# marbl/parsnp

Hardware: AMD Instinct MI355X
Metric: genomes/sec (MUM+LCB end-to-end) (higher is better)
Workload: dtype int32

## Files before the change

### parsnp_amd/csrc/engine/engine_core.h

```cpp
#pragma once
#include <algorithm>
#include <atomic>
#include <chrono>
#include <cstdint>
#include <cstdio>
#include <cstdlib>
#include <cstring>
#include <memory>
#include <mutex>
#include <new>
#include <string>
#include <thread>
#include <vector>

#include "kernels.h"
#include "store_kernels.h"
#include "dense_kernels.h"
#include "index_kernels.h"

namespace pm {

struct HostPool {
    void* (*alloc_fn)(size_t) = nullptr;
    void (*free_fn)(void*) = nullptr;
    struct Block { void* p = nullptr; size_t cap = 0; };
    std::vector<Block> idle;
    std::mutex mu;
    Block take(size_t n) {
        std::lock_guard<std::mutex> lk(mu);
        size_t best = idle.size();
        for (size_t i = 0; i < idle.size(); i++)
            if (idle[i].cap >= n && (best == idle.size() || idle[i].cap < idle[best].cap)) best = i;
        if (best != idle.size() && idle[best].cap <= 2 * n + (1u << 20)) { Block b = idle[best]; idle.erase(idle.begin() + (long)best); return b; }
        Block b; b.cap = n + n / 8 + 256; b.p = alloc_fn(b.cap);
        if (!b.p) throw std::bad_alloc();
        return b;
    }
    void give(Block b) { std::lock_guard<std::mutex> lk(mu); if (b.p) idle.push_back(b); }
    ~HostPool() { for (auto& b : idle) free_fn(b.p); }
};

struct ClearJob { void* p; size_t bytes; int value; };
struct BatchResult {
    int64_t nregions = 0, total = 0;
    int nq = 0;
    std::vector<int64_t> off;
    HostPool::Block kb, lonb, spb, fwdb;
    HostPool::Block startb, strandb, flagsb;
    bool rows = false, dirty_known = false;
    int64_t table_id = 0;
    int64_t store_base = -1;
    std::shared_ptr<HostPool> pool;
    int32_t* start() const { return (int32_t*)startb.p; }
    uint8_t* strand() const { return (uint8_t*)strandb.p; }
    const uint32_t* flags() const { return (const uint32_t*)flagsb.p; }
    const int32_t* k() const { return (const int32_t*)kb.p; }
    const int32_t* lon() const { return (const int32_t*)lonb.p; }
    const int32_t* sp() const { return (const int32_t*)spb.p; }
    const uint8_t* fwd() const { return (const uint8_t*)fwdb.p; }
    void release() {
        if (pool) { pool->give(kb); pool->give(lonb); pool->give(spb); pool->give(fwdb); pool->give(startb); pool->give(strandb); pool->give(flagsb); }
        kb = lonb = spb = fwdb = startb = strandb = flagsb = HostPool::Block();
    }
    BatchResult() = default;
    BatchResult(const BatchResult&) = delete;
    BatchResult& operator=(const BatchResult&) = delete;
    ~BatchResult() { release(); }
};

struct PhaseTime { const char* name; float ms; };

struct Collectives {
    int rank = 0, world = 1;
    int (*allreduce_min_i32)(void* ctx, int32_t* buf, int64_t count) = nullptr;
    int (*allgather)(void* ctx, const void* send, int64_t send_bytes, void* recv) = nullptr;
    void* ctx = nullptr;
    bool device = false;
};

inline int bits_for(uint64_t v) { int b = 1; while (b < 64 && (v >> b)) b++; return b; }

template <class B>
class Engine {
public:
    explicit Engine(B& backend) : be(backend), pool(std::make_shared<HostPool>()) { pool->alloc_fn = &B::host_alloc; pool->free_fn = &B::host_free; }
    std::shared_ptr<HostPool> pool;
    ~Engine() { release(); }

    std::string error;
    std::vector<PhaseTime> timing;
    int64_t last_events = 0, last_candidates = 0, last_rest = 0, last_positions = 0, last_accepted = 0;
    double last_alg[3] = {0, 0, 0};
    uint64_t alg_raw[3] = {0, 0, 0};
    uint64_t alg_sets[8 * kAlgSets] = {};

    int ngen = 0;
    bool want_rows = false;
    std::vector<int64_t> glen_h;
    Collectives coll;
    int g_first = 1, g_last = 1;
    void set_shard(const Collectives& c) { coll = c; }
    static void shard_range(int n, int rank, int world, int* first, int* last) {
        int q = n - 1;
        *first = 1 + (int)((int64_t)q * rank / world);
        *last = 1 + (int)((int64_t)q * (rank + 1) / world);
    }

    int load_genomes(int n, const uint8_t* const* seqs, const int64_t* lens) {
        const bool dbg = getenv("PARSNP_DEBUG_TIMERS") != nullptr;
        auto now = [] { return std::chrono::duration<double>(std::chrono::steady_clock::now().time_since_epoch()).count(); };
        double tl = now();
        auto lap = [&](const char* what) { if (dbg) { be.sync(); const double t = now(); fprintf(stderr, "[upload] %-14s %.4f s\n", what, t - tl); tl = t; } };
        ngen = n;
        glen_h.assign(lens, lens + n);
        shard_range(n, coll.rank, coll.world, &g_first, &g_last);
        auto resident = [&](int) { return true; };
        std::vector<int64_t> goff(2 * (size_t)n);
        int64_t words = 2;
        int64_t maxlen = 0;
        for (int g = 0; g < n; g++) {
            if (!resident(g)) { goff[2 * (size_t)g] = goff[2 * (size_t)g + 1] = 64; continue; }
            maxlen = std::max(maxlen, lens[g]);
            for (int s = 0; s < 2; s++) {
                goff[2 * (size_t)g + s] = words * 32;
                words += (lens[g] + 31) / 32 + 2;
            }
        }
        words += 8;
        total_words = words;
        blk = (SeqBlock*)be.alloc((size_t)words * sizeof(SeqBlock));
        d_goff = (int64_t*)be.alloc(sizeof(int64_t) * 2 * (size_t)n);
        d_glen = (int64_t*)be.alloc(sizeof(int64_t) * (size_t)n);
        if (!blk || !d_goff || !d_glen) { error = "device allocation failed (genomes)"; return -3; }
        lap("allocate");
        be.memset(blk, 0, (size_t)words * sizeof(SeqBlock));
        be.h2d(d_goff, goff.data(), sizeof(int64_t) * goff.size());
        be.h2d(d_glen, lens, sizeof(int64_t) * (size_t)n);
        std::vector<char> res((size_t)n, 0);
        for (int g = 0; g < n; g++) res[(size_t)g] = resident(g) && lens[g] > 0;
        lap("clear + tables");
        if (!be.stage_genomes(n, seqs, lens, res, goff, blk, maxlen)) { error = "genome upload failed: " + be.error(); return -3; }
        lap("stage + pack");
        P = Packed{blk, d_goff, d_glen};
        return 0;
    }

    std::vector<int64_t> mumi_covered;
    struct GapBatch {
        const int64_t* ref_start = nullptr; const int64_t* ref_len = nullptr;
        const int32_t* store_ids = nullptr;
    };
    int run(int64_t nreg, const int64_t* starts, const int64_t* lens, const int32_t* minsize, BatchResult* out, bool want_events = false,
            bool mumi = false, const GapBatch* gb = nullptr) {
        budget_exceeded = false;
        dense_mode = false; dense_h.clear(); last_dense_regions = 0; last_dense_overrun_ms = -1;
        const int64_t ordinal = call_ordinal;
        if (dense_all && nreg > 0) { dense_h.assign((size_t)nreg, 1); dense_mode = true; }
        const auto t0 = std::chrono::steady_clock::now();
        index_rebuild = false;
        int rc = run_once(nreg, starts, lens, minsize, out, want_events, mumi, gb);
        if (rc == kIndexRebuild) {
            (void)be.collect();
            call_ordinal = ordinal;
            index_rebuild = true;
            rc = run_once(nreg, starts, lens, minsize, out, want_events, mumi, gb);
        }
        if (rc == -5 && budget_exceeded && !dense_mode) {
            budget_retries++;
            last_dense_overrun_ms = (float)std::chrono::duration<double, std::milli>(std::chrono::steady_clock::now() - t0).count();
            dense_h.resize((size_t)nreg);
            be.d2h(dense_h.data(), d_dense.p, (size_t)nreg);
            (void)be.collect();
            call_ordinal = ordinal;
            dense_mode = true; budget_exceeded = false;
            rc = run_once(nreg, starts, lens, minsize, out, want_events, mumi, gb);
            if (rc == kIndexRebuild) {
                (void)be.collect();
                call_ordinal = ordinal;
                index_rebuild = true;
                rc = run_once(nreg, starts, lens, minsize, out, want_events, mumi, gb);
            }
        }
        dense_mode = false; index_rebuild = false;
        return rc;
    }
    bool dense_all = false;
    int64_t last_dense_regions = 0;
    float last_dense_overrun_ms = -1;
    int dense_rounds = 0;
    int64_t anchor_table_id = 0, anchor_table_rows = 0;
    bool budget_exceeded = false;
    long budget_retries = 0;
    static constexpr int kIndexRebuild = -99;
    bool index_rebuild = false;
    int64_t index_overflow_seen = 0;
    int run_once(int64_t nreg, const int64_t* starts, const int64_t* lens, const int32_t* minsize, BatchResult* out, bool want_events,
                 bool mumi, const GapBatch* gb = nullptr) {
        timing.clear();
        const int nq = ngen - 1;
        out->nregions = nreg; out->nq = nq; out->total = 0;
        out->off.assign((size_t)nreg + 1, 0);
        out->release();
        out->pool = pool;
        if (nreg == 0) return 0;
        if (nq < 1) { error = "need at least one query genome"; return -2; }
        const int no_small = mumi ? 1 : 0;

        const size_t nrow = (size_t)nreg * (size_t)ngen;
        const size_t regz = (size_t)nreg;
        const size_t bytes_R = sizeof(RegionInfo) * regz, bytes_pre = 8 * (regz + 1);
        const bool from_store = gb && gb->store_ids;
        if (gb && !from_store) { error = "bad region list"; return -2; }
        const size_t nrow_staged = gb ? 0 : nrow;
        uint8_t* block = (uint8_t*)be.staging(bytes_R + 2 * bytes_pre + 16 * nrow_staged + (gb ? 4 * regz : 0) + 64);
        if (!block) { error = "cannot allocate the request staging block"; return -3; }
        RegionInfo* R = (RegionInfo*)block;
        int64_t* posbase = (int64_t*)(block + bytes_R);
        int64_t* cbase = posbase + regz + 1;
        int64_t* stage = cbase + regz + 1;
        std::vector<size_t> guess_r(regz, 0);
        std::vector<int64_t> units_r(regz, 0);
        if (from_store) {
            for (int64_t r = 0; r < nreg; r++) {
                if (gb->store_ids[r] < 0 || gb->store_ids[r] >= rg_count) { error = "region outside the region store"; return -2; }
                if (gb->ref_start[r] < 0 || gb->ref_len[r] < 0 || gb->ref_start[r] + gb->ref_len[r] > glen_h[0]) { error = "region outside its genome"; return -2; }
                if (gb->ref_len[r] >= (1ll << 31)) { error = "region longer than 2^31"; return -5; }
            }
            memcpy(stage, gb->store_ids, sizeof(int32_t) * regz);
        } else {
            const int nt = (int)std::max<int64_t>(1, std::min<int64_t>(8, nreg / 512));
            std::vector<int> bad((size_t)nt, 0);
            auto part = [&](int t) {
                const int64_t r0 = nreg * t / nt, r1 = nreg * (t + 1) / nt;
                for (int64_t r = r0; r < r1; r++) {
                    const int64_t* st = starts + r * ngen; const int64_t* ln = lens + r * ngen;
                    const int minlen = minsize[r] < 1 ? 1 : minsize[r];
                    const int div = std::max(8, minlen);
                    const int K = minlen < kMaxK ? minlen : kMaxK, stride = minlen - K + 1;
                    const int64_t nR = ln[0];
                    size_t gs = 0;
                    int64_t units = 0;
                    int b = 0;
                    for (int g = 0; g < ngen; g++) {
                        if (st[g] < 0 || ln[g] < 0 || st[g] + ln[g] > glen_h[(size_t)g]) b |= 1;
                        if (ln[g] >= (1ll << 31)) b |= 2;
                        if (!g) continue;
                        gs += (size_t)(2 * ln[g] / div);
                        int64_t ns = (ln[g] >= K && nR >= K && g >= g_first && g < g_last) ? (ln[g] - K) / stride + 1 : 0;
                        if (small_pair(nR, ln[g]) && !no_small) ns = 0;
                        units += (ns + kUnitSamples - 1) / kUnitSamples;
                    }
                    guess_r[(size_t)r] = gs; units_r[(size_t)r] = units;
                    bad[(size_t)t] |= b;
                    memcpy(stage + r * ngen, st, sizeof(int64_t) * (size_t)ngen);
                    memcpy(stage + nrow + r * ngen, ln, sizeof(int64_t) * (size_t)ngen);
                }
            };
            if (nt == 1) part(0);
            else {
                std::vector<std::thread> th;
                for (int t = 1; t < nt; t++) th.emplace_back(part, t);
                part(0);
                for (auto& x : th) x.join();
            }
            int b = 0;
            for (int x : bad) b |= x;
            if (b & 1) { error = "region outside its genome"; return -2; }
            if (b & 2) { error = "region longer than 2^31"; return -5; }
        }
        int64_t npos = 0, tsize = 0, fwords = 0, nunits = 0;
        int64_t tsize_b = 0, fwords_b = 0, nbk = 0, npos_bucketed = 0;
        std::vector<int64_t> bbase(regz + 1, 0);
        const bool by_index_buckets = index_build && !index_rebuild;
        int32_t max_nr = 1;
        size_t ev_guess = 1 << 16;
        cbase[0] = 0;
        for (int64_t r = 0; r < nreg; r++) {
            RegionInfo& ri = R[(size_t)r];
            ri.ref_pos = gb ? gb->ref_start[r] : starts[r * ngen];
            ri.nR = (int32_t)(gb ? gb->ref_len[r] : lens[r * ngen]);
            ri.minsize = minsize[r];
            ri.minlen = minsize[r] < 1 ? 1 : minsize[r];
            ri.K = ri.minlen < kMaxK ? ri.minlen : kMaxK;
            ri.stride = ri.minlen - ri.K + 1;
            int64_t slots = 16;
            while (slots < slot_factor * (int64_t)ri.nR) slots <<= 1;
            ri.tmask = (uint32_t)(slots - 1);
            int64_t fbits = 64;
            while (fbits < filter_factor * (int64_t)ri.nR) fbits <<= 1;
            ri.fmask = (uint32_t)(fbits - 1);
            const int ls = bits_for((uint64_t)slots) - 1, lf = bits_for((uint64_t)fbits) - 1;
            const int sb = std::min(kBucketBits, ls - 1), fb = lf - (ls - sb);
            const bool bucketed = by_index_buckets && slots >= index_bucket_min && fb >= 5 && fb <= kBucketFilterBits;
            ri.pad_ = bucketed ? (uint32_t)sb | ((uint32_t)fb << 8) | kBucketed : (uint32_t)ls | ((uint32_t)std::min(lf, 29) << 8);
            bbase[(size_t)r] = nbk;
            if (bucketed) { nbk += slots >> sb; npos_bucketed += ri.nR; }
            ri.tbase = bucketed ? -1 - tsize_b : tsize; (bucketed ? tsize_b : tsize) += slots;
            ri.fbase = bucketed ? -1 - fwords_b : fwords; (bucketed ? fwords_b : fwords) += fbits / 32;
            ri.posbase = npos; posbase[(size_t)r] = npos; npos += ri.nR;
            cbase[(size_t)r + 1] = cbase[(size_t)r] + (((int64_t)ri.nR + kChunkPos - 1) >> kCoarseShift) + 1;
            max_nr = std::max(max_nr, ri.nR);
            ev_guess += guess_r[(size_t)r];
            nunits += units_r[(size_t)r];
        }
        posbase[regz] = npos;
        bbase[regz] = nbk;
        const int64_t tsize_clear = tsize, fwords_clear = fwords;
        for (int64_t r = 0; r < nreg; r++) {
            RegionInfo& ri = R[(size_t)r];
            if (ri.tbase < 0) { ri.tbase = tsize_clear + (-1 - ri.tbase); ri.fbase = fwords_clear + (-1 - ri.fbase); }
        }
        tsize += tsize_b; fwords += fwords_b;
        last_index_bucketed = npos_bucketed; last_index_overflow = index_rebuild ? index_overflow_seen : 0; last_index_lost = -1;
        last_positions = npos; last_candidates = 0; last_accepted = 0; last_grouped = 0; last_grouped_wide = 0; last_handed_back = -1; last_wide_regions = 0;
        const int64_t npairs = nreg * nq;
        const int64_t nchunks = cbase[regz] - nreg;
        const int64_t centries = cbase[regz] * nq;
        const int lbits = bits_for((uint64_t)max_nr);
        if (bits_for((uint64_t)npairs) + lbits + 1 > 64) { error = "batch too large for 64-bit event keys"; return -5; }
        if (npairs >= (1ll << 31) || nreg >= (1ll << 31)) { error = "too many regions in one batch"; return -5; }
        if (nunits >= (1ll << 31)) { error = "too many work units in one batch"; return -5; }
        if (centries >= (1ll << 31)) { error = "coarse event index too large"; return -5; }

        be.mark("setup");
        ensure(d_R, regz);
        ensure(d_starts, nrow); ensure(d_lens, nrow);
        ensure(d_posbase, regz + 1); ensure(d_cbase, regz + 1);
        be.h2d_staged(d_R.p, R, bytes_R);
        be.h2d_staged(d_posbase.p, posbase, bytes_pre);
        be.h2d_staged(d_cbase.p, cbase, bytes_pre);
        if (!gb) {
            be.h2d_staged(d_starts.p, stage, sizeof(int64_t) * nrow);
            be.h2d_staged(d_lens.p, stage + nrow, sizeof(int64_t) * nrow);
        } else if (from_store) {
            ensure(d_list, regz);
            be.h2d_staged(d_list.p, stage, sizeof(int32_t) * regz);
            be.launch("gather_regions", (int64_t)nrow, GatherRegions{d_list.p, ngen, d_rg_start.p, d_rg_len.p, d_starts.p, d_lens.p});
        }
        const size_t ncounter = (size_t)kSlices * kSliceStride + 8;
        ensure(d_counter, ncounter);
        uint32_t* d_err = (uint32_t*)(d_counter.p + (size_t)kSlices * kSliceStride);

        ensure(d_slots, (size_t)tsize); ensure(d_filter, (size_t)fwords);
        ensure(d_next, (size_t)std::max<int64_t>(npos, 1)); ensure(d_rep, (size_t)std::max<int64_t>(npos, 1));
        ensure(d_epm, (size_t)std::max<int64_t>(npos, 1) + 1);
        const int64_t nwv = (npos + 63) / 64;
        const bool from_store_ = gb && gb->store_ids;
        ensure(d_repeated, (size_t)(npos / 32 + 2));
        ensure(d_ucount, (size_t)npairs + 1); ensure(d_uoff, (size_t)npairs + 1);
        ensure(d_coarse, (size_t)std::max<int64_t>(centries, 1));
        ensure(d_wmask, (size_t)nwv + 1); ensure(d_wcount, (size_t)nwv + 1); ensure(d_woff, (size_t)nwv + 1);
        if (from_store_) ensure(d_alg, 8 * (size_t)kAlgSets);
        ensure(d_dense, regz);
        {
            const ClearJob jobs[] = {
                {d_filter.p, sizeof(uint32_t) * (size_t)fwords_clear, 0}, {d_slots.p, sizeof(uint64_t) * (size_t)tsize_clear, 0xff}, {d_counter.p, 8 * ncounter, 0},
                {d_repeated.p, 4 * (size_t)(npos / 32 + 2), 0}, {d_coarse.p, 4 * (size_t)std::max<int64_t>(centries, 1), 0},
                {d_ucount.p + npairs, 8, 0}, {d_wcount.p + nwv, 8, 0}, {from_store_ ? d_alg.p : nullptr, from_store_ ? (size_t)64 * kAlgSets : 0, 0},
                {dense_mode ? nullptr : d_dense.p, dense_mode ? 0 : regz, 0}};
            be.clear_many(jobs, (int)(sizeof jobs / sizeof jobs[0]));
        }
        int64_t nflag = 0;
        if (dense_mode) {
            for (int64_t r = 0; r < nreg; r++) nflag += dense_h[(size_t)r] ? 1 : 0;
            be.h2d(d_dense.p, dense_h.data(), regz);
            last_dense_regions = nflag;
        }
        if (gb) be.launch("check_rows", (int64_t)nrow, CheckRows{d_R.p, d_starts.p, d_lens.p, ngen, d_glen, d_err});
        last_alg[0] = last_alg[1] = last_alg[2] = 0;
        if (from_store) {
            be.launch_wave("alg_bytes", (nreg * nq + kAlgPairs - 1) / kAlgPairs, AlgBytes{d_R.p, d_lens.p, ngen, nreg * nq, d_alg.p});
        }
        be.mark("index");
        const size_t kOvfSlot = (size_t)kSlices * kSliceStride + 6, kLostSlot = kOvfSlot + 1;
        const uint64_t ovf_cap = nbk > 0 ? (uint64_t)(index_overflow_cap > 0 ? index_overflow_cap : npos_bucketed / 32 + 1024) : 0;
        if (nbk > 0) {
            const int pbits = bits_for((uint64_t)npos), bbits = bits_for((uint64_t)nbk);
            if (pbits + bbits > 64) { error = "batch too large for 64-bit index keys"; return -5; }
            ensure(d_bkbase, regz + 1); ensure(d_ikey, (size_t)npos); ensure(d_ikey2, (size_t)npos); ensure(d_bkbegin, (size_t)nbk + 1); ensure(d_ovf, (size_t)ovf_cap);
            be.h2d(d_bkbase.p, bbase.data(), 8 * (regz + 1));
            be.launch("index_keys", npos, IndexKeys{P, d_R.p, nreg, d_posbase.p, d_bkbase.p, pbits, d_ikey.p, d_next.p, d_rep.p});
            if (!sort_keys_on(be, d_ikey.p, d_ikey2.p, (size_t)npos, pbits, pbits + bbits, 0)) {
                ensure(d_ikey3, (size_t)npos); ensure(d_ikey4, (size_t)npos);
                be.launch("index_key_buckets", npos, IndexKeyBuckets{d_ikey.p, pbits, d_ikey3.p});
                be.sort_pairs(d_ikey3.p, d_ikey4.p, d_ikey.p, d_ikey2.p, (size_t)npos, bbits);
            }
            be.launch("index_bucket_bounds", nbk + 1, IndexBucketBounds{d_ikey2.p, npos, pbits, d_bkbegin.p});
            be.launch_wave("index_bucket_fill", nbk, IndexBucketFill{P, d_R.p, nreg, d_bkbase.p, d_ikey2.p, d_bkbegin.p, pbits, d_slots.p, d_filter.p, d_next.p, d_rep.p,
                                                                     d_counter.p + kOvfSlot, d_ovf.p, ovf_cap});
            be.launch("index_overflow", (int64_t)ovf_cap, IndexOverflow{P, d_R.p, nreg, d_posbase.p, d_counter.p + kOvfSlot, d_ovf.p, ovf_cap, d_slots.p, d_next.p, d_rep.p});
        }
        if (npos_bucketed < npos) be.launch("index_insert", npos, IndexInsert{P, d_R.p, nreg, d_posbase.p, d_slots.p, d_next.p, d_filter.p, d_rep.p});
        if (index_verify) be.launch("index_verify", npos, IndexVerify{P, d_R.p, nreg, d_posbase.p, d_slots.p, d_filter.p, d_next.p, d_counter.p + kLostSlot});
        bool index_counts_read = false;
        be.mark("repeat");
        ensure(d_run, (size_t)std::max<int64_t>(npos, 1));
        be.launch("run_length", npos, RunLength{P, d_R.p, nreg, d_posbase.p, d_run.p});
        be.launch("repeat_length", npos, RepeatLength{P, d_R.p, nreg, d_posbase.p, d_slots.p, d_filter.p, d_next.p, d_run.p, d_rep.p, d_repeated.p, d_err, work_budget, d_dense.p});
        if (nflag > 0) {
            be.mark("dense_sa");
            if (int rc = dense_build(R, nreg, nflag)) return rc;
        }

        be.mark("units");
        be.launch("count_units", npairs, CountUnits{d_R.p, d_lens.p, ngen, d_ucount.p, g_first, g_last, no_small});
        be.exclusive_scan(d_ucount.p, d_uoff.p, (size_t)npairs + 1);
        if (!gb && nreg == 1) call_ordinal = 0; else if (gb) call_ordinal++;
        const size_t ord = gb || nreg == 1 ? (size_t)call_ordinal : (size_t)-1;
        if (ord != (size_t)-1 && call_hints.size() <= ord) call_hints.resize(ord + 1);
        CallHint none;
        CallHint& hint = ord != (size_t)-1 ? call_hints[ord] : none;
        if (hint_shrink > 1) {
            if (hint.units > 0) hint.units = std::max<int64_t>(1, hint.units / hint_shrink);
            if (hint.ncand > 0) hint.ncand = std::max<int64_t>(1, hint.ncand / hint_shrink);
        }
        bool units_known = !gb;
        if (gb && !(fast_tail && hint.units > 0)) {
            be.d2h(&nunits, d_uoff.p + npairs, 8);
            units_known = true;
        } else if (gb) nunits = hint.units + hint.units / 8 + 64;
        if (nunits >= (1ll << 31)) { error = "too many work units in one batch"; return -5; }
        if (gb) ev_guess += (size_t)nunits * 16;

        ensure(d_sliceoff, (size_t)kSlices + 1);
        uint64_t nev = 0;
        size_t slice_cap = (std::min<size_t>(std::max<size_t>(ev_cap_hint, ev_guess), (size_t)1 << 31) + kSlices - 1) / kSlices + 64;
        std::vector<uint64_t> counts(ncounter);
        uint32_t errbits = 0;
        ensure(d_qcount, (size_t)kSlices * kSliceStride);
        size_t queue_cap = std::max<size_t>(std::max<size_t>(rest_cap_hint[nreg == 1], (size_t)nunits * kUnitSamples / 16 / kSlices), 64) + 64;
        uint64_t nrest = 0;
        uint32_t sticky = 0;
        std::vector<uint64_t> qcounts((size_t)kSlices * kSliceStride);
        const bool small_groups = group_small && !no_small && !want_events && nreg >= 2;
        const bool first_form = small_groups && nq <= kGrpGenomes;
        const bool wide_form = small_groups && group_wide && nq <= kWideGenomes;
        const bool grouping = first_form || wide_form;
        const size_t kGrpSlot = (size_t)kSlices * kSliceStride + 2;
        const size_t kWideSlot = kGrpSlot + 1;
        size_t grp_cap = grouping ? std::max<size_t>(grp_cap_hint, (size_t)npairs * 3) + 64 : 0;
        uint64_t ngrp = 0;
        if (grouping) { ensure(d_gflag, (size_t)nreg); ensure(d_glo, (size_t)npairs); }
        int64_t nunits_live = nunits;
        uint64_t worst_slice = 0;
        for (bool again = false;; again = true) {
            ensure(d_units, (size_t)std::max<int64_t>(nunits, 1));
            be.launch("fill_units", nunits, FillUnits{P, d_starts.p, d_lens.p, ngen, d_uoff.p, d_ucount.p, npairs, d_units.p});
            ensure(d_evkey, slice_cap * kSlices); ensure(d_evval, slice_cap * kSlices); ensure(d_rest, queue_cap * kSlices);
            if (again) be.memset(d_counter.p, 0, 8 * ncounter);
            if (grouping) {
                ensure(d_evkey3, grp_cap + ev_cap_hint); ensure(d_evval3, grp_cap + ev_cap_hint);
                ensure(d_state, grp_cap + ev_cap_hint); ensure(d_emax, grp_cap + ev_cap_hint);
                be.mark("grouped_events");
                if (first_form)
                    be.launch_wave("grouped_pair_events", xcd_grid(nreg),
                                   GroupedPairEvents{P, d_R.p, d_starts.p, d_lens.p, ngen, d_rep.p, d_evkey3.p, d_evval3.p, d_counter.p + kGrpSlot, (uint64_t)grp_cap, lbits,
                                                     d_glo.p, g_first, g_last, d_gflag.p, d_state.p, d_emax.p, d_epm.p, (int64_t)nreg});
                if (wide_form)
                    be.launch_wave("grouped_pair_events_wide", xcd_grid(nreg),
                                   GroupedPairEventsWide{P, d_R.p, d_starts.p, d_lens.p, ngen, d_rep.p, d_evkey3.p, d_evval3.p, d_counter.p + kGrpSlot, (uint64_t)grp_cap, lbits,
                                                         d_glo.p, g_first, g_last, d_gflag.p, d_state.p, d_emax.p, d_epm.p, (int64_t)nreg, first_form ? 1 : 0, d_counter.p + kWideSlot});
            }
            be.memset(d_qcount.p, 0, 8 * (size_t)kSlices * kSliceStride);
            be.mark("seed_extend");
            be.launch("seed_extend", nunits * 64,
                      SeedExtend{P, d_R.p, d_units.p, d_slots.p, d_filter.p, d_next.p, d_rep.p, d_repeated.p,
                                 d_evkey.p, d_evval.p, d_counter.p, (uint64_t)slice_cap, lbits, d_err, work_budget, d_rest.p, d_qcount.p, (uint64_t)queue_cap, d_uoff.p + npairs});
            if (nunits > 0)
                be.launch("seed_rest", (int64_t)(queue_cap * kSlices),
                          SeedRest{P, d_R.p, d_units.p, d_rest.p, d_qcount.p, (uint64_t)queue_cap, d_slots.p, d_filter.p, d_next.p, d_rep.p,
                                   d_evkey.p, d_evval.p, d_counter.p, (uint64_t)slice_cap, lbits, d_err, work_budget, d_dense.p});
            if (nunits > 0 && nflag > 0) {
                be.mark("dense_search");
                be.launch("seed_dense", (int64_t)(queue_cap * kSlices),
                          SeedDense{P, d_R.p, d_units.p, d_rest.p, d_qcount.p, (uint64_t)queue_cap, d_dfi.p, d_dstart.p, d_dval2.p, d_rep.p,
                                    d_evkey.p, d_evval.p, d_counter.p, (uint64_t)slice_cap, lbits});
                be.mark("seed_extend");
            }
            if (!no_small)
                be.launch("small_pair_events", npairs * 2,
                          SmallPairEvents{P, d_R.p, d_starts.p, d_lens.p, ngen, d_rep.p, d_evkey.p, d_evval.p, d_counter.p, (uint64_t)slice_cap, lbits, g_first, g_last, grouping ? d_gflag.p : nullptr});
            be.mark("sort");
            be.launch_wave("slice_offsets", 1, SliceOffsets{d_counter.p, d_sliceoff.p});
            group_downloads();
            be.d2h_async(qcounts.data(), d_qcount.p, 8 * qcounts.size());
            if (from_store) be.d2h_async(alg_sets, d_alg.p, sizeof alg_sets);
            if (!units_known) be.d2h_async(&nunits_live, d_uoff.p + npairs, 8);
            run_beside();
            be.d2h(counts.data(), d_counter.p, 8 * counts.size());
            if (!index_counts_read) {
                index_counts_read = true;
                if (nbk > 0) last_index_overflow = (int64_t)counts[kOvfSlot];
                if (index_verify) last_index_lost = (int64_t)counts[kLostSlot];
                if (nbk > 0 && counts[kOvfSlot] > ovf_cap) { index_overflow_seen = (int64_t)counts[kOvfSlot]; return kIndexRebuild; }
            }
            if (!units_known) {
                units_known = true;
                if (nunits_live >= (1ll << 31)) { error = "too many work units in one batch"; return -5; }
                if (nunits_live > nunits) {
                    nunits = nunits_live;
                    queue_cap = std::max<size_t>(queue_cap, (size_t)nunits * kUnitSamples / 16 / kSlices + 64);
                    tail_repeats++;
                    continue;
                }
            }
            uint64_t worst = 0, qworst = 0;
            nev = 0; nrest = 0;
            for (int sl = 0; sl < kSlices; sl++) {
                const uint64_t c = counts[(size_t)sl * kSliceStride]; nev += c; worst = std::max(worst, c);
                const uint64_t q = qcounts[(size_t)sl * kSliceStride]; nrest += q; qworst = std::max(qworst, q);
            }
            errbits = (uint32_t)counts[(size_t)kSlices * kSliceStride];
            ngrp = grouping ? counts[kGrpSlot] : 0;
            worst_slice = worst;
            if (worst <= slice_cap && qworst <= queue_cap && ngrp <= grp_cap) break;
            if (ngrp > grp_cap) grp_cap = (size_t)(ngrp + ngrp / 8 + 64);
            if (worst > slice_cap) slice_cap = (size_t)(worst + worst / 8 + 64);
            if (qworst > queue_cap) queue_cap = (size_t)(qworst + qworst / 8 + 64);
            sticky |= errbits & (kErrWork | kErrRows);
        }
        errbits |= sticky;
        if (from_store) {
            alg_raw[0] = alg_raw[1] = alg_raw[2] = 0;
            for (int x = 0; x < kAlgSets; x++) for (int k = 0; k < 3; k++) alg_raw[k] += alg_sets[8 * x + k];
        }
        if (from_store) { last_alg[0] = (double)alg_raw[0] / 4.0; last_alg[1] = (double)alg_raw[1] / 2.0; last_alg[2] = (double)alg_raw[2] / 2.0; }
        if (errbits & kErrRows) { error = "region outside its genome"; return -2; }
        rest_cap_hint[nreg == 1] = queue_cap - 64;
        if (gb) hint.units = std::max<int64_t>(nunits_live, 1);
        last_rest = (int64_t)nrest;
        ev_cap_hint = (size_t)(nev + nev / 4);
        if (grouping) grp_cap_hint = (size_t)(ngrp + ngrp / 4);
        last_events = (int64_t)(nev + ngrp);
        last_grouped = (int64_t)ngrp;
        last_grouped_wide = wide_form ? (int64_t)counts[kWideSlot] : 0;
        last_handed_back = wide_form ? (int64_t)counts[kWideSlot + 1] : -1;
        last_wide_regions = wide_form ? (int64_t)counts[kWideSlot + 2] : 0;
        const bool sharded = coll.world > 1 || coll.device;
        if ((errbits & kErrWork) && !sharded) { budget_exceeded = true; error = "per-thread work budget exceeded (degenerate repeat structure in a region)"; return -5; }

        ensure(d_evkey2, std::max<size_t>(nev, 1)); ensure(d_evval2, std::max<size_t>(nev, 1));
        ensure_keep(d_evkey3, std::max<size_t>(ngrp + nev, 1), (size_t)ngrp); ensure_keep(d_evval3, std::max<size_t>(ngrp + nev, 1), (size_t)ngrp);
        const int keybits = bits_for((uint64_t)npairs) + lbits + 1;
        uint64_t *skey = d_evkey3.p, *sval = d_evval3.p;
        const int64_t nbuckets = (int64_t)nq * nchunks;
        const bool by_buckets = bucket_sort && nev > 0 && nbuckets < ((int64_t)1 << 31);
        ensure(d_lo, (size_t)npairs + 1);
        if (by_buckets) {
            ensure(d_bcount, (size_t)nbuckets + 1); ensure(d_bbegin, (size_t)nbuckets + 1); ensure(d_pbase, (size_t)npairs);
            int shift = 6;
            while (((uint64_t)1 << shift) < worst_slice) shift++;
            be.memset(d_bcount.p, 0, 8 * ((size_t)nbuckets + 1));
            be.launch("pair_bucket_base", npairs, PairBucketBase{nq, d_cbase.p, d_pbase.p});
            be.launch("event_bucket_count", (int64_t)kSlices << shift, EventBucketCount{d_evkey.p, d_counter.p, (uint64_t)slice_cap, shift, lbits, d_pbase.p, d_bcount.p});
            be.exclusive_scan(d_bcount.p, d_bbegin.p, (size_t)nbuckets + 1);
            be.launch("event_place", (int64_t)kSlices << shift,
                      EventPlace{d_evkey.p, d_evval.p, d_counter.p, (uint64_t)slice_cap, shift, lbits, d_pbase.p, d_bbegin.p, d_bcount.p, d_evkey3.p + ngrp, d_evval3.p + ngrp});
            be.launch("event_order", nbuckets, EventOrder{d_bbegin.p, nbuckets, d_evkey3.p + ngrp, d_evval3.p + ngrp});
        } else if (nev > 0) {
            be.launch("compact_events", (int64_t)nev, CompactEvents{d_evkey.p, d_evval.p, d_sliceoff.p, (uint64_t)slice_cap, d_evkey2.p, d_evval2.p});
            be.sort_pairs(d_evkey2.p, d_evkey3.p + ngrp, d_evval2.p, d_evval3.p + ngrp, (size_t)nev, keybits);
        }
        be.mark("scan");
        const int64_t nev_sorted = (int64_t)nev;
        nev += ngrp;
        if (by_buckets) be.launch("coarse_from_buckets", centries, CoarseFromBuckets{d_bbegin.p, d_cbase.p, nreg, nq, (int64_t)ngrp, d_coarse.p, d_lo.p, npairs, nev_sorted});
        else be.launch("pair_bounds", npairs, PairBounds{skey, (int64_t)nev, lbits, npairs, d_lo.p, (int64_t)ngrp});
        if (grouping) be.launch("grouped_bounds", npairs, GroupedBounds{d_gflag.p, d_glo.p, nq, d_lo.p});
        ensure_keep(d_state, std::max<size_t>(nev, 1), (size_t)ngrp); ensure_keep(d_emax, std::max<size_t>(nev, 1), (size_t)ngrp);
        const int64_t nsorted = (int64_t)(nev - ngrp);
        if (nsorted > 0) {
            const int64_t nwaves = (nsorted + kWaveEvents - 1) / kWaveEvents;
            ensure(d_wsummary, (size_t)nwaves);
            const WaveScanCore core{skey + ngrp, sval + ngrp, nsorted, lbits, d_R.p, nq, d_rep.p};
            be.launch_wave("wave_summary", nwaves, WaveSummary{core, d_wsummary.p});
            be.launch_wave("wave_scan", nwaves, WaveScan{core, d_wsummary.p, d_lo.p, (int64_t)ngrp, d_state.p + ngrp, d_emax.p + ngrp});
        }

        if (want_events) {
            ev_key_h.resize((size_t)nev); ev_val_h.resize((size_t)nev); rep_h.resize((size_t)npos);
            if (nev) { be.d2h(ev_key_h.data(), skey, 8 * (size_t)nev); be.d2h(ev_val_h.data(), sval, 8 * (size_t)nev); }
            if (npos) be.d2h(rep_h.data(), d_rep.p, 4 * (size_t)npos);
            ev_lbits = lbits;
        }

        if (mumi) {
            be.mark("mumi_coverage");
            ensure(d_cov, (size_t)npairs);
            be.launch("mumi_coverage", npairs, MumiCoverage{d_R.p, skey, sval, d_lo.p, d_state.p, d_rep.p, lbits, ngen, d_cov.p});
            mumi_covered.resize((size_t)npairs);
            be.d2h(mumi_covered.data(), d_cov.p, 8 * (size_t)npairs);
            if (sharded) {
                int widest = 0;
                for (int r = 0; r < coll.world; r++) { int a, b; shard_range(ngen, r, coll.world, &a, &b); widest = std::max(widest, b - a); }
                const size_t per = (size_t)std::max(widest, 1) + 1;
                std::vector<int64_t> send(per, 0), recv(per * (size_t)coll.world);
                for (int g = g_first; g < g_last; g++) send[(size_t)(g - g_first)] = mumi_covered[(size_t)(g - 1)];
                send[per - 1] = errbits;
                if (allgather_host(send.data(), (int64_t)(8 * send.size()), recv.data())) { error = "all-gather of MUMi coverage failed"; return -4; }
                for (int r = 0; r < coll.world; r++) {
                    int a, b; shard_range(ngen, r, coll.world, &a, &b);
                    for (int g = a; g < b; g++) mumi_covered[(size_t)(g - 1)] = recv[(size_t)r * per + (size_t)(g - a)];
                    errbits |= (uint32_t)recv[(size_t)r * per + per - 1];
                }
                if (errbits & kErrWork) { budget_exceeded = true; error = "per-thread work budget exceeded on some rank (degenerate repeat structure in a region)"; return -5; }
            }
            be.mark(nullptr);
            collect_timing();
            return 0;
        }

        be.mark("master_ep");
        if (!by_buckets) be.launch("coarse_fill", (int64_t)nev, CoarseFill{skey, (int64_t)nev, lbits, d_lo.p, d_R.p, d_cbase.p, nq, d_coarse.p});
        else if (ngrp > 0) be.launch("coarse_fill", (int64_t)ngrp, CoarseFill{skey, (int64_t)ngrp, lbits, d_lo.p, d_R.p, d_cbase.p, nq, d_coarse.p});
        if (master_seg) be.launch_wave("master_ep_seg", xcd_grid(nchunks), MasterEPSeg{d_R.p, nreg, ngen, skey, d_lo.p, d_emax.p, lbits, d_epm.p, d_cbase.p, d_coarse.p, g_first, g_last, grouping ? d_gflag.p : nullptr, nchunks});
        else be.launch_wave("master_ep", xcd_grid(nchunks), MasterEP{d_R.p, nreg, ngen, skey, d_lo.p, d_emax.p, lbits, d_epm.p, d_cbase.p, d_coarse.p, g_first, g_last, grouping ? d_gflag.p : nullptr, nchunks});
        int32_t verdict = 0;
        if (sharded && coll.device) {
            be.mark("exchange_ep");
            be.fill32(d_epm.p + npos, (errbits & kErrWork) ? -1 : 0);
            if (be.allreduce_min_i32_dev(d_epm.p, npos + 1)) { error = "RCCL all-reduce of Master.EP failed: " + be.error(); return -4; }
            be.d2h_async(&verdict, d_epm.p + npos, 4);
        } else if (sharded) {
            be.mark("exchange_ep");
            std::vector<int32_t> h((size_t)npos + 1);
            if (npos) be.d2h(h.data(), d_epm.p, 4 * (size_t)npos);
            h[(size_t)npos] = (errbits & kErrWork) ? -1 : 0;
            if (coll.allreduce_min_i32(coll.ctx, h.data(), npos + 1)) { error = "all-reduce of Master.EP failed"; return -4; }
            verdict = h[(size_t)npos];
            if (verdict >= 0 && npos) be.h2d(d_epm.p, h.data(), 4 * (size_t)npos);
        }
        be.mark("candidates");
        be.launch_wave("cand_mark", nwv, CandMark{d_R.p, nreg, d_posbase.p, npos, d_epm.p, d_wmask.p, d_wcount.p});
        be.exclusive_scan(d_wcount.p, d_woff.p, (size_t)nwv + 1);
        const int64_t* ncand_p = d_woff.p + nwv;
        const bool anchor_guess = nreg == 1 && !gb && hint.nok >= dirty_min;
        const bool may_skip_waits = !sharded && want_rows && resident && hint.ncand > 0 && (from_store || anchor_guess) && fast_tail;
        for (int attempt = may_skip_waits ? 0 : 1;; attempt++) {
            const bool exact = attempt > 0;
            int64_t ncand_i = 0;
            if (exact) be.d2h(&ncand_i, ncand_p, 8);
            if (verdict < 0) { budget_exceeded = true; error = "per-thread work budget exceeded on some rank (degenerate repeat structure in a region)"; return -5; }
            if (exact) {
                last_candidates = ncand_i;
                if (ncand_i == 0) { hint.ncand = 1; hint.nok = 0; if (resident && from_store) out->store_base = ms_count; be.mark(nullptr); collect_timing(); return 0; }
            }
            const uint64_t ncand = exact ? (uint64_t)ncand_i : (uint64_t)(hint.ncand + hint.ncand / 8 + 256);
            ensure(d_cand, (size_t)ncand);
            be.launch("cand_write", nwv * 64, CandWrite{d_R.p, nreg, d_posbase.p, d_wmask.p, d_woff.p, d_cand.p, ncand});
            const uint64_t* scand = d_cand.p;

            be.mark("fold");
            ensure(d_ok, (size_t)ncand); ensure(d_ok_k, (size_t)ncand); ensure(d_ok_lon, (size_t)ncand);
            ensure(d_osp, (size_t)ncand * (size_t)nq); ensure(d_ofwd, (size_t)ncand * (size_t)nq);
            const GenomeAtK* at = nullptr;
            if (sharded) {
                ensure(d_at, (size_t)ncand * (size_t)nq);
                be.launch("state_at_candidate", (int64_t)ncand * nq, StateAtCandidate{d_R.p, scand, ngen, skey, sval, d_lo.p, d_state.p, d_rep.p, lbits, d_at.p, d_cbase.p, d_coarse.p});
                be.mark("exchange_states");
                const size_t nqz = (size_t)nq, cz = (size_t)ncand;
                int widest = 0;
                for (int r = 0; r < coll.world; r++) { int a, b; shard_range(ngen, r, coll.world, &a, &b); widest = std::max(widest, b - a); }
                widest = std::max(widest, 1);
                const size_t blk = cz * (size_t)widest;
                if (coll.device) {
                    ensure(d_xsend, blk); ensure(d_xrecv, blk * (size_t)coll.world);
                    be.launch("pack_states", (int64_t)blk, PackStates{d_at.p, nq, g_first - 1, g_last - g_first, widest, d_xsend.p});
                    if (be.allgather_dev(d_xsend.p, (int64_t)(sizeof(GenomeAtK) * blk), d_xrecv.p)) { error = "RCCL all-gather of candidate states failed: " + be.error(); return -4; }
                    be.launch("unpack_states", (int64_t)(cz * nqz), UnpackStates{d_xrecv.p, nq, coll.world, widest, (int64_t)ncand, d_at.p});
                } else {
                    std::vector<GenomeAtK> all(cz * nqz);
                    be.d2h(all.data(), d_at.p, sizeof(GenomeAtK) * all.size());
                    std::vector<GenomeAtK> send(blk), recv(blk * (size_t)coll.world);
                    const size_t mine = (size_t)(g_last - g_first);
                    for (size_t c = 0; c < cz; c++)
                        for (size_t x = 0; x < mine; x++) send[c * (size_t)widest + x] = all[c * nqz + (size_t)(g_first - 1) + x];
                    if (coll.allgather(coll.ctx, send.data(), (int64_t)(sizeof(GenomeAtK) * send.size()), recv.data())) { error = "all-gather of candidate states failed"; return -4; }
                    for (int r = 0; r < coll.world; r++) {
                        int a, b; shard_range(ngen, r, coll.world, &a, &b);
                        const GenomeAtK* src = recv.data() + (size_t)r * send.size();
                        for (size_t c = 0; c < cz; c++)
                            for (int x = 0; x < b - a; x++) all[c * nqz + (size_t)(a - 1 + x)] = src[c * (size_t)widest + (size_t)x];
                    }
                    be.h2d(d_at.p, all.data(), sizeof(GenomeAtK) * all.size());
                }
                be.mark("fold");
                at = d_at.p;
            }
            be.launch_wave("fold_candidates", xcd_grid((int64_t)ncand),
                           FoldCandidates{d_R.p, scand, ngen, at, skey, sval, d_lo.p, d_state.p, d_rep.p, lbits, d_cbase.p, d_coarse.p,
                                          d_ok_k.p, d_ok_lon.p, d_osp.p, d_ofwd.p, d_ok.p, (int64_t)ncand, ncand_p});

            be.mark("compact");
            ensure(d_okcnt, (size_t)ncand + 1); ensure(d_okpos, (size_t)ncand + 1);
            be.launch("ok_count", (int64_t)ncand + 1, OkCount{d_ok.p, ncand_p, d_okcnt.p, (int64_t)ncand});
            be.exclusive_scan(d_okcnt.p, d_okpos.p, (size_t)ncand + 1);
            const int64_t* nok_p = d_okpos.p + ncand;
            int64_t nok = 0;
            if (exact) be.d2h(&nok, nok_p, 8);
            const size_t nokz = exact ? (size_t)nok : (size_t)ncand, nqz2 = (size_t)nq, ngz = (size_t)ngen;
            ensure(d_creg, std::max<size_t>(nokz, 1)); ensure(d_ck, std::max<size_t>(nokz, 1)); ensure(d_clon, std::max<size_t>(nokz, 1));
            std::vector<int32_t> reg_h(nokz);
            out->release();
            out->kb = pool->take(4 * nokz); out->lonb = pool->take(4 * nokz);
            out->rows = want_rows; out->dirty_known = false; out->table_id = 0; out->store_base = -1;
            const int64_t ms_before = ms_count, rg_before = rg_count, lay_before = layout_rows, pkey_before = rg_pkey_init;
            bool anchor_call = false;
            if (!want_rows) {
                ensure(d_csp, std::max<size_t>(nokz * nqz2, 1)); ensure(d_cfwd, std::max<size_t>(nokz * nqz2, 1));
                be.launch("compact_sp", (int64_t)ncand * nq,
                          CompactSp{scand, d_ok.p, d_okpos.p, nq, d_ok_k.p, d_ok_lon.p, d_osp.p, d_ofwd.p, d_creg.p, d_ck.p, d_clon.p, d_csp.p, d_cfwd.p, ncand_p});
                be.mark("download");
                group_downloads();
                out->spb = pool->take(4 * nokz * nqz2); out->fwdb = pool->take(nokz * nqz2);
                be.d2h_async(out->spb.p, d_csp.p, 4 * nokz * nqz2);
                be.d2h_async(out->fwdb.p, d_cfwd.p, nokz * nqz2);
            } else {
                anchor_call = nreg == 1 && !gb && (exact ? nok >= dirty_min : anchor_guess);
                const bool keep_rows = resident && (anchor_call || from_store);
                const bool to_store = anchor_call || keep_rows;
                int32_t* p_start; uint8_t* p_strand; int32_t* p_lon; uint32_t* p_flags;
                if (to_store) {
                    if (anchor_call) { ms_count = 0; rg_count = 0; layout_rows = -1; rg_pkey_init = 0; }
                    const size_t base = (size_t)ms_count, upto = base + nokz;
                    ensure_keep(d_anchor_start, std::max<size_t>(upto * ngz, 1), base * ngz); ensure_keep(d_ms_strand, std::max<size_t>(upto * ngz, 1), base * ngz);
                    ensure_keep(d_anchor_lon, std::max<size_t>(upto, 1), base); ensure_keep(d_anchor_flags, std::max<size_t>(upto, 1), base);
                    ensure_keep(d_ms_shift, std::max<size_t>(upto, 1), base); ensure_keep(d_ms_len, std::max<size_t>(upto, 1), base); ensure_keep(d_ms_state, std::max<size_t>(upto, 1), base);
                    p_start = d_anchor_start.p + base * ngz; p_strand = d_ms_strand.p + base * ngz; p_lon = d_anchor_lon.p + base; p_flags = d_anchor_flags.p + base;
                    out->store_base = (int64_t)base;
                    ms_count = (int64_t)upto;
                } else {
                    ensure(d_csp, std::max<size_t>(nokz * ngz, 1)); ensure(d_cfwd, std::max<size_t>(nokz * ngz, 1)); ensure(d_cflags, std::max<size_t>(nokz, 1));
                    p_start = d_csp.p; p_strand = d_cfwd.p; p_lon = d_clon.p; p_flags = d_cflags.p;
                }
                const bool long_list = nreg == 1 && (exact ? nok >= dirty_min : anchor_guess);
                if (long_list) ensure(d_dirty, nokz);
                {
                    const ClearJob jobs[] = {{p_flags, 4 * nokz, 0}, {long_list ? d_dirty.p : nullptr, long_list ? 4 * nokz : 0, 0},
                                             {to_store ? d_ms_shift.p + (ms_count - (int64_t)nokz) : nullptr, to_store ? 4 * nokz : 0, 0},
                                             {to_store ? d_ms_state.p + (ms_count - (int64_t)nokz) : nullptr, to_store ? nokz : 0, 0}};
                    be.clear_many(jobs, 4);
                }
                be.launch("compact_candidates", (int64_t)ncand * ngen,
                          CompactCandidates{scand, d_ok.p, d_okpos.p, ngen, d_ok_k.p, d_ok_lon.p, d_osp.p, d_ofwd.p, d_starts.p, d_lens.p, d_glen,
                                            d_creg.p, d_ck.p, p_lon, p_start, p_strand, p_flags, ncand_p});
                if (long_list) {
                    const int64_t nblocks = ((int64_t)nokz + kDirtyBlock - 1) / kDirtyBlock, groups = (ngen + 63) / 64;
                    ensure(d_bmax, (size_t)nblocks * ngz); ensure(d_bmin, (size_t)nblocks * ngz);
                    be.launch_wave("dirty_extent", nblocks * groups, DirtyExtent{p_start, p_lon, p_flags, nok_p, ngen, d_bmax.p, d_bmin.p});
                    be.launch_wave("dirty_prefix", groups, DirtyPrefix{nblocks, ngen, d_bmax.p, d_bmin.p});
                    be.launch_wave("dirty_mark", nblocks * groups, DirtyMark{p_start, p_lon, nok_p, ngen, d_bmax.p, d_bmin.p, p_flags, d_dirty.p});
                    be.launch("dirty_merge", (int64_t)nokz, DirtyMerge{d_dirty.p, p_flags, nok_p});
                    out->dirty_known = true;
                }
                if (to_store) {
                    be.d2d(d_ms_len.p + (ms_count - (int64_t)nokz), p_lon, 4 * nokz);
                    if (anchor_call) out->table_id = ++table_counter;
                }
                be.mark("download");
                group_downloads();
                out->flagsb = pool->take(4 * nokz);
                be.d2h_async(out->flagsb.p, p_flags, 4 * nokz);
                if (!keep_rows) {
                    out->startb = pool->take(4 * nokz * ngz); out->strandb = pool->take(nokz * ngz);
                    be.d2h_async(out->startb.p, p_start, 4 * nokz * ngz);
                    be.d2h_async(out->strandb.p, p_strand, nokz * ngz);
                }
                be.d2h_async(out->lonb.p, p_lon, 4 * nokz);
            }
            if (!want_rows) be.d2h_async(out->lonb.p, d_clon.p, 4 * nokz);
            be.d2h_async(reg_h.data(), d_creg.p, 4 * nokz);
            be.d2h_async(out->kb.p, d_ck.p, 4 * nokz);
            int64_t counts_h[2] = {ncand_i, nok};
            if (!exact) { be.d2h_async(&counts_h[0], ncand_p, 8); be.d2h_async(&counts_h[1], nok_p, 8); }
            flush_downloads();
            be.mark(nullptr);
            be.sync();
            if (!exact) {
                ncand_i = counts_h[0]; nok = counts_h[1];
                const bool fits = (uint64_t)ncand_i <= ncand && anchor_call == (nreg == 1 && !gb && nok >= dirty_min);
                if (!fits) {
                    ms_count = ms_before; rg_count = rg_before; layout_rows = lay_before; rg_pkey_init = pkey_before;
                    tail_repeats++;
                    be.mark("candidates");
                    continue;
                }
                last_candidates = ncand_i;
                if (out->store_base >= 0) ms_count = out->store_base + nok;
            }
            hint.ncand = std::max<int64_t>(ncand_i, 1); hint.nok = nok;
            last_accepted = nok;
            if (anchor_call) { anchor_table_rows = nok; anchor_table_id = out->table_id; }
            for (int64_t w = 0; w < nok; w++) out->off[(size_t)reg_h[(size_t)w] + 1]++;
            for (int64_t r = 0; r < nreg; r++) out->off[(size_t)r + 1] += out->off[(size_t)r];
            out->total = out->off[(size_t)nreg];
            if (out->table_id && out->store_base == 0) anchor_flags_h.assign(out->flags(), out->flags() + nok);
            break;
        }
        collect_timing();
        return 0;
    }


    bool resident = false;
    int64_t ms_count = 0;
    int64_t rg_count = 0;
    std::vector<RegInfo> rg_info_h;
    std::vector<uint32_t> anchor_flags_h;
    static constexpr int kAgain = -6;

    void begin_store_call() { timing.clear(); last_events = last_rest = last_positions = last_candidates = last_accepted = last_grouped = last_grouped_wide = last_wide_regions = 0; last_handed_back = -1; last_index_bucketed = last_index_overflow = 0; last_index_lost = -1; last_alg[0] = last_alg[1] = last_alg[2] = 0; }
    Store store_view() { return Store{d_anchor_start.p, d_ms_strand.p, d_anchor_lon.p, d_anchor_flags.p, d_ms_shift.p, d_ms_len.p, d_ms_state.p, ngen}; }
    Layout layout_view(uint64_t* image, bool coherent = true) { return Layout{image, d_lay_off.p, d_lay_bits.p, coherent ? 1 : 0}; }
    size_t layout_geometry() {
        const size_t ngz = (size_t)ngen;
        if (lay_words == 0) {
            std::vector<int64_t> off(ngz + 1, 0), bits(ngz);
            for (size_t j = 0; j < ngz; j++) { bits[j] = glen_h[j] + 1; off[j + 1] = off[j] + (bits[j] + 63) / 64 + 1; }
            ensure(d_lay_off, ngz + 1); ensure(d_lay_bits, ngz);
            be.h2d(d_lay_off.p, off.data(), 8 * (ngz + 1)); be.h2d(d_lay_bits.p, bits.data(), 8 * ngz);
            lay_words = (size_t)off[ngz];
            lay_off_h = off;
        }
        return lay_words;
    }
    int need_resident(int64_t table_id) {
        if (!resident) { error = "the session is not in resident mode"; return -2; }
        if (table_id == 0 || table_id != anchor_table_id) { error = "the anchor table of this request is no longer resident"; return -2; }
        return 0;
    }
    int store_settle(int64_t table_id, RowInfo* out) {
        if (int rc = settle_launch(table_id)) return rc;
        return store_info(0, anchor_table_rows, out);
    }
    int settle_launch(int64_t table_id) {
        if (int rc = need_resident(table_id)) return rc;
        begin_store_call();
        const int64_t rows = anchor_table_rows;
        const size_t words = layout_geometry();
        ensure(d_image, words);
        be.mark("settle");
        ensure(d_foreign_count, 2);
        be.memset(d_foreign_count.p, 0, 16);
        ms_key_rows = 0; foreign_seen = 0;
        be.memset(d_image.p, 0, 8 * words);
        ensure(d_recwords, words);
        be.memset(d_recwords.p, 0, words);
        const Store S = store_view();
        const Layout L = layout_view(d_image.p);
        be.launch_wave("settle_clean", rows, SettleClean{S, P});
        std::vector<int32_t> fl;
        for (int64_t c = 0; c < rows; c++) { const uint32_t f = anchor_flags_h[(size_t)c]; if (!(f & (kRowBad | kRowOutside)) && (f & kRowDirty)) fl.push_back((int32_t)c); }
        const bool many_flagged = flagged_div > 1 && fl.size() * (size_t)flagged_div > (size_t)rows;
        bool ordered = true;
        for (int64_t c = 0; c < rows && ordered; c++) { const uint32_t f = anchor_flags_h[(size_t)c]; ordered = !((f & kRowEarly) && !(f & (kRowBad | kRowOutside | kRowDirty))); }
        if (ordered && !force_atomic_marks) be.launch_wave("store_mark_ordered", ((rows + kMarkRows - 1) / kMarkRows) * ((ngen + 63) / 64), StoreMarkOrdered{S, L, rows});
        else be.launch("store_mark", rows * ngen, StoreMark{S, L, 0, (uint8_t)(kStAccepted | kStFlagged), kStAccepted});
        be.launch("layout_sentinel", (int64_t)ngen, LayoutSentinel{d_lay_off.p, d_lay_bits.p, d_image.p});
        if (!fl.empty()) {
            const uint64_t* before_once = d_once.p; const uint64_t* before_twice = d_twice.p;
            ensure(d_once, words); ensure(d_twice, words); ensure(d_list, fl.size());
            if (d_once.p != before_once || d_twice.p != before_twice) { be.memset(d_once.p, 0, 8 * words); be.memset(d_twice.p, 0, 8 * words); }
            be.h2d(d_list.p, fl.data(), 4 * fl.size());
            be.launch("collide_mark", (int64_t)fl.size() * ngen, CollideMark{S, d_list.p, layout_view(d_once.p), d_twice.p});
            be.launch_wave("collide_test", (int64_t)fl.size(), CollideTest{S, d_list.p, layout_view(d_twice.p, false)});
            be.launch("collide_clear", (int64_t)fl.size() * ngen, CollideClear{S, d_list.p, layout_view(d_once.p), d_twice.p});
            ensure(d_t_rem, 2); ensure(d_t_done, fl.size());
            {
                const ClearJob jobs[] = {{d_t_rem.p, 16, 0}, {d_t_done.p, fl.size(), 0}};
                be.clear_many(jobs, 2);
            }
            be.launch("count_tangled", (int64_t)fl.size(), CountTangled{S, d_list.p, d_t_rem.p});
            if (many_flagged) {
                uint64_t tangled = 0;
                be.d2h(&tangled, d_t_rem.p, 8);
                if ((int64_t)tangled > tangled_max) {
                    be.mark(nullptr);
                    collect_timing_more();
                    error = "too many rows of the list overlap one another (rearranged genomes): the host route decides";
                    return kAgain;
                }
            }
            be.launch_wave("settle_flagged", (int64_t)fl.size(), SettleFlagged{S, layout_view(d_image.p, false), P, d_list.p});
            {
                const int32_t* before = d_owner.p;
                ensure(d_owner, words);
                if (d_owner.p != before) be.memset(d_owner.p, 0, 4 * words);
            }
            int rounds = tangle_rounds ? kTangleRounds : 0;
            if (rounds && tangle_ran > 0) {
                int last = 0;
                for (int r = 1; r < tangle_ran; r++) if (tangle_left[r] < tangle_left[r - 1]) last = r;
                rounds = std::min(kTangleRounds, last + 2);
            }
            ensure(d_t_left, kTangleRounds);
            for (int round = 0; round < rounds; round++) {
                be.launch_wave("tangle_owner", (int64_t)fl.size(), TangleOwner{S, d_list.p, d_lay_off.p, d_lay_bits.p, d_owner.p, d_t_done.p, d_t_rem.p});
                be.launch_wave("tangle_settle", (int64_t)fl.size(), TangleSettle{S, layout_view(d_image.p, false), P, d_list.p, d_owner.p, d_t_done.p, d_t_rem.p});
                be.launch_wave("tangle_clear", (int64_t)fl.size(), TangleClear{S, d_list.p, d_lay_off.p, d_lay_bits.p, d_owner.p, d_t_done.p, d_t_rem.p, d_t_left.p + round});
            }
            tangle_ran = 0;
            if (rounds) { be.d2h_async(tangle_left, d_t_left.p, 8 * (size_t)rounds); tangle_ran = rounds; }
            be.launch_wave("settle_tangled", 1, SettleTangled{S, L, P, d_list.p, (int64_t)fl.size(), d_t_done.p, d_t_rem.p});
        }
        layout_rows = rows;
        return 0;
    }
    int store_settle_seeds(int64_t table_id, int32_t q, RowInfo* out, std::vector<RegInfo>* infos, std::vector<int32_t>* ids) {
        infos->clear(); ids->clear();
        if (int rc = settle_launch(table_id)) return rc;
        const int64_t rows = anchor_table_rows;
        rg_count = 0;
        if (rows == 0) return 0;
        const Store S = store_view();
        ensure(d_rowinfo, (size_t)rows);
        be.launch("store_info", rows, StoreInfoOut{S, 0, d_rowinfo.p});
        be.mark("seeds");
        ensure(d_ch_flag, (size_t)rows + 1); ensure(d_ch_pos, (size_t)rows + 1); ensure(d_list, (size_t)rows);
        ensure(d_sd_cnt, (size_t)rows + 1); ensure(d_sd_off, (size_t)rows + 1); ensure(d_sd_keep, (size_t)rows);
        be.launch("chain_flag", rows + 1, ChainFlag{S, rows, d_ch_flag.p});
        be.exclusive_scan(d_ch_flag.p, d_ch_pos.p, (size_t)rows + 1);
        be.launch("anchor_list", rows, AnchorList{S, d_ch_pos.p, d_list.p});
        const int64_t* nacc = d_ch_pos.p + rows;
        const Layout L = layout_view(d_image.p, false);
        be.memset(d_sd_cnt.p + rows, 0, 8);
        be.launch_wave("seed_count", xcd_grid(rows), SeedCount{S, L, P, d_list.p, nacc, q, d_sd_cnt.p, d_sd_keep.p, rows});
        be.exclusive_scan(d_sd_cnt.p, d_sd_off.p, (size_t)rows + 1);
        size_t cap = std::max<size_t>(rg_cap_hint, (size_t)rows / 4 + 1024);
        std::vector<RegInfo> raw;
        for (bool again = false;; again = true) {
            ensure(d_rg_start, cap * (size_t)ngen); ensure(d_rg_len, cap * (size_t)ngen); ensure(d_rg_info, cap);
            be.launch_wave("seed_place", xcd_grid(rows), SeedPlace{S, L, P, d_list.p, nacc, d_sd_off.p, d_sd_keep.p, d_rg_start.p, d_rg_len.p, d_rg_info.p, (uint64_t)cap, rows});
            be.mark(nullptr);
            const size_t guess = std::min(cap, rg_cap_hint / (size_t)hint_shrink);
            raw.resize(guess);
            group_downloads();
            if (guess) be.d2h_async(raw.data(), d_rg_info.p, sizeof(RegInfo) * guess);
            if (!again) be.d2h_async(out, d_rowinfo.p, sizeof(RowInfo) * (size_t)rows);
            int64_t got = 0;
            be.d2h(&got, d_sd_off.p + rows, 8);
            if ((size_t)got <= cap) {
                rg_count = got;
                raw.resize((size_t)got);
                if ((size_t)got > guess) be.d2h(raw.data() + guess, d_rg_info.p + guess, sizeof(RegInfo) * ((size_t)got - guess));
                break;
            }
            cap = (size_t)got + (size_t)got / 8 + 64;
            be.mark("seeds");
        }
        rg_cap_hint = (size_t)rg_count + (size_t)rg_count / 4;
        if (rg_info_h.size() < (size_t)rg_count) rg_info_h.resize((size_t)rg_count);
        bool sorted = true;
        for (int64_t i = 0; i < rg_count; i++) { rg_info_h[(size_t)i] = raw[(size_t)i]; if (i && raw[(size_t)i - 1].key >= raw[(size_t)i].key) sorted = false; }
        if (!sorted) { error = "seed regions out of order"; return -4; }
        infos->swap(raw);
        ids->resize((size_t)rg_count);
        for (int64_t i = 0; i < rg_count; i++) (*ids)[(size_t)i] = (int32_t)i;
        collect_timing_more();
        return 0;
    }
    int store_info(int64_t first, int64_t count, RowInfo* out) {
        if (!resident || first < 0 || count < 0 || first + count > ms_count) { error = "rows outside the MUM store"; return -2; }
        if (count == 0) return 0;
        ensure(d_rowinfo, (size_t)count);
        be.launch("store_info", count, StoreInfoOut{store_view(), first, d_rowinfo.p});
        be.mark(nullptr);
        be.d2h(out, d_rowinfo.p, sizeof(RowInfo) * (size_t)count);
        collect_timing_more();
        return 0;
    }
    void take_regions(int64_t first, int64_t upto, std::vector<RegInfo>* infos, std::vector<int32_t>* ids) {
        const size_t m = (size_t)(upto - first);
        std::vector<RegInfo> raw(m);
        if (m) be.d2h(raw.data(), d_rg_info.p + first, sizeof(RegInfo) * m);
        if (rg_info_h.size() < (size_t)upto) rg_info_h.resize((size_t)upto);
        std::vector<int32_t> order;
        for (size_t i = 0; i < m; i++) { rg_info_h[(size_t)first + i] = raw[i]; if (raw[i].key >= 0) order.push_back((int32_t)i); }
        std::sort(order.begin(), order.end(), [&](int32_t x, int32_t y) { return raw[(size_t)x].key < raw[(size_t)y].key; });
        infos->clear(); ids->clear();
        for (int32_t i : order) { infos->push_back(raw[(size_t)i]); ids->push_back((int32_t)(first + i)); }
    }
    int store_seeds(int64_t table_id, const int32_t* acc, int64_t nacc, int32_t q, std::vector<RegInfo>* infos, std::vector<int32_t>* ids) {
        if (int rc = need_resident(table_id)) return rc;
        if (layout_rows < 0) { error = "the anchor list has not been settled"; return -2; }
        for (int64_t i = 0; i < nacc; i++) if (acc[i] < 0 || acc[i] >= anchor_table_rows) { error = "anchor outside the table"; return -2; }
        rg_count = 0;
        infos->clear(); ids->clear();
        begin_store_call();
        if (nacc == 0) return 0;
        ensure(d_list, (size_t)nacc); ensure(d_rg_count, 2);
        be.h2d(d_list.p, acc, 4 * (size_t)nacc);
        be.mark("seeds");
        size_t cap = std::max<size_t>(rg_cap_hint, (size_t)nacc / 4 + 1024);
        for (;;) {
            ensure(d_rg_start, cap * (size_t)ngen); ensure(d_rg_len, cap * (size_t)ngen); ensure(d_rg_info, cap);
            be.memset(d_rg_count.p, 0, 16);
            be.launch_wave("seed_walk", xcd_grid(nacc), SeedWalk{store_view(), layout_view(d_image.p, false), P, d_list.p, q, d_rg_start.p, d_rg_len.p, d_rg_info.p, d_rg_count.p, (uint64_t)cap, (int64_t)nacc});
            uint64_t got = 0;
            be.d2h(&got, d_rg_count.p, 8);
            if (got <= cap) { rg_count = (int64_t)got; break; }
            cap = (size_t)got + (size_t)got / 8 + 64;
        }
        rg_cap_hint = (size_t)rg_count + (size_t)rg_count / 4;
        be.mark(nullptr);
        take_regions(0, rg_count, infos, ids);
        collect_timing_more();
        return 0;
    }
    int store_regions_equal(const int32_t* a, const int32_t* b, int64_t n, uint8_t* same) {
        if (!resident) { error = "the session is not in resident mode"; return -2; }
        for (int64_t i = 0; i < n; i++) if (a[i] < 0 || a[i] >= rg_count || b[i] < 0 || b[i] >= rg_count) { error = "region outside the region store"; return -2; }
        if (n == 0) return 0;
        ensure(d_list, (size_t)n); ensure(d_list2, (size_t)n); ensure(d_small8, (size_t)n);
        be.h2d(d_list.p, a, 4 * (size_t)n); be.h2d(d_list2.p, b, 4 * (size_t)n);
        be.launch_wave("regions_equal", n, RegionsEqual{d_list.p, d_list2.p, ngen, d_rg_start.p, d_rg_len.p, d_small8.p});
        be.d2h(same, d_small8.p, (size_t)n);
        return 0;
    }
    void (*beside_fn)(void*) = nullptr; void* beside_ctx = nullptr;
    void run_beside() { if (beside_fn) { void (*f)(void*) = beside_fn; beside_fn = nullptr; f(beside_ctx); } }
    int store_search(const int32_t* ids, const int32_t* minsize, int64_t n, int64_t* first_row, int64_t* off, void (*beside)(void*) = nullptr, void* ctx = nullptr) {
        beside_fn = beside; beside_ctx = ctx;
        struct Always { Engine* e; ~Always() { e->run_beside(); } } on_every_way_out{this};
        if (!resident) { error = "the session is not in resident mode"; return -2; }
        std::vector<int64_t> rs((size_t)n), rl((size_t)n);
        for (int64_t i = 0; i < n; i++) {
            if (ids[i] < 0 || ids[i] >= rg_count) { error = "region outside the region store"; return -2; }
            rs[(size_t)i] = rg_info_h[(size_t)ids[i]].ref_start; rl[(size_t)i] = rg_info_h[(size_t)ids[i]].ref_len;
        }
        *first_row = ms_count;
        off[0] = 0;
        if (n == 0) return 0;
        GapBatch gb;
        gb.store_ids = ids; gb.ref_start = rs.data(); gb.ref_len = rl.data();
        BatchResult br;
        const bool keep = want_rows;
        want_rows = true;
        const int rc = run(n, nullptr, nullptr, minsize, &br, false, false, &gb);
        want_rows = keep;
        if (rc) return rc;
        *first_row = br.store_base >= 0 ? br.store_base : ms_count;
        for (int64_t i = 0; i <= n; i++) off[i] = br.off[(size_t)i];
        return 0;
    }
    int store_validate(const int32_t* regions, const int64_t* row0, const int32_t* cnt, int64_t nreg, const int64_t* cluster_first, int64_t ncl, int32_t q,
                       uint32_t* trouble, std::vector<RegInfo>* kids, std::vector<int32_t>* kid_ids, int64_t info_first = 0, int64_t info_count = 0, RowInfo* info = nullptr,
                       int64_t stage_first = 0, int32_t* second_stage_ran = nullptr, int32_t generation_no = 1, int32_t* done = nullptr) {
        if (!resident || layout_rows < 0) { error = "the anchor list has not been settled"; return -2; }
        kids->clear(); kid_ids->clear(); *trouble = 0;
        if (nreg == 0 || ncl == 0) return 0;
        int64_t total = 0;
        for (int64_t x = 0; x < nreg; x++) {
            if (regions[x] < 0 || regions[x] >= rg_count || row0[x] < 0 || cnt[x] < 0 || row0[x] + cnt[x] > ms_count) { error = "bad generation list"; return -2; }
            total += cnt[x];
        }
        if (cluster_first[0] != 0 || cluster_first[ncl] != nreg) { error = "bad cluster list"; return -2; }
        if (stage_first < 0 || stage_first >= ncl) { error = "bad stage boundary"; return -2; }
        begin_store_call();
        const size_t cap = (size_t)rg_count + 2 * (size_t)total + 16;
        ensure_keep(d_rg_start, cap * (size_t)ngen, (size_t)rg_count * (size_t)ngen); ensure_keep(d_rg_len, cap * (size_t)ngen, (size_t)rg_count * (size_t)ngen);
        ensure_keep(d_rg_info, cap, (size_t)rg_count);
        const size_t bytes = 4 * (size_t)nreg + 8 * (size_t)nreg + 4 * (size_t)nreg + 8 * ((size_t)ncl + 1) + 64;
        uint8_t* block = (uint8_t*)be.staging(bytes);
        if (!block) { error = "cannot allocate the request staging block"; return -3; }
        int64_t* s_row0 = (int64_t*)block; int64_t* s_first = s_row0 + nreg; int32_t* s_reg = (int32_t*)(s_first + ncl + 1); int32_t* s_cnt = s_reg + nreg;
        memcpy(s_row0, row0, 8 * (size_t)nreg); memcpy(s_first, cluster_first, 8 * ((size_t)ncl + 1)); memcpy(s_reg, regions, 4 * (size_t)nreg); memcpy(s_cnt, cnt, 4 * (size_t)nreg);
        ensure(d_v_row0, (size_t)nreg); ensure(d_v_first, (size_t)ncl + 1); ensure(d_list, (size_t)nreg); ensure(d_list2, (size_t)nreg); ensure(d_rg_count, 4);
        ensure(d_v_done, (size_t)ncl); ensure(d_v_defer, (size_t)ncl); ensure(d_v_involved, (size_t)ncl);
        be.h2d_staged(d_v_row0.p, s_row0, 8 * (size_t)nreg); be.h2d_staged(d_v_first.p, s_first, 8 * ((size_t)ncl + 1));
        be.h2d_staged(d_list.p, s_reg, 4 * (size_t)nreg); be.h2d_staged(d_list2.p, s_cnt, 4 * (size_t)nreg);
        foreign_cap = std::min<size_t>((size_t)1 << 16, ((size_t)32 << 20) / (8 * (size_t)ngen));
        ensure(d_foreign, foreign_cap); ensure(d_foreign_masks, foreign_cap * (size_t)ngen); ensure(d_foreign_count, 2);
        ensure_keep(d_ms_key, (size_t)ms_count, (size_t)ms_key_rows); ms_key_rows = ms_count;
        if (rg_pkey_init > rg_count) rg_pkey_init = 0;
        ensure_keep(d_rg_pkey, cap, (size_t)rg_pkey_init);
        if (rg_pkey_init < rg_count) { be.memset(d_rg_pkey.p + rg_pkey_init, 0, 8 * (size_t)(rg_count - rg_pkey_init)); rg_pkey_init = rg_count; }
        constexpr size_t kOutwCap = 4096; constexpr int64_t kOutwWaves = 256;
        ensure(d_outw, kOutwCap); ensure(d_outw_count, 2);
        const int64_t na = stage_first > 0 ? stage_first : ncl;
        uint64_t head[4] = {(uint64_t)rg_count, 0, 0, 0};
        if (info_count > 0) {
            if (info_first < 0 || info_first + info_count > ms_count) { error = "rows outside the MUM store"; return -2; }
            ensure(d_rowinfo, (size_t)info_count);
        }
        std::vector<int32_t> done_h((size_t)ncl, 0);
        auto generation = [&](bool exact) {
            be.h2d(d_rg_count.p, head, 32);
            be.memset(d_v_done.p, 0, 4 * (size_t)ncl);
            be.memset(d_outw_count.p, 0, 16);
            const uint8_t* defer = nullptr;
            if (exact) {
                be.memset(d_v_defer.p, 0, (size_t)ncl);
                const int64_t c0 = stage_first > 0 ? na : 0, cn = ncl - c0;
                if (cn >= 2) {
                    const size_t words = layout_geometry();
                    const uint64_t* b1 = d_once.p; const uint64_t* b2 = d_twice.p; const int32_t* b3 = d_owner.p;
                    ensure(d_once, words); ensure(d_twice, words); ensure(d_owner, words);
                    if (d_once.p != b1 || d_twice.p != b2) { be.memset(d_once.p, 0, 8 * words); be.memset(d_twice.p, 0, 8 * words); }
                    if (d_owner.p != b3) be.memset(d_owner.p, 0, 4 * words);
                    be.launch_wave("cluster_extents", cn, ClusterExtents{ngen, d_rg_start.p, d_rg_len.p, d_list.p, d_v_first.p, layout_view(d_once.p), d_twice.p, d_owner.p, c0, 1});
                    be.launch_wave("cluster_involved", cn, ClusterInvolved{ngen, d_rg_start.p, d_rg_len.p, d_list.p, d_v_first.p, layout_view(d_twice.p, false), d_owner.p, d_v_involved.p, c0});
                    be.launch_wave("cluster_defer", cn, ClusterDefer{ngen, d_rg_start.p, d_rg_len.p, d_list.p, d_v_first.p, d_lay_off.p, d_lay_bits.p, d_owner.p, d_v_involved.p, d_v_defer.p, c0});
                    be.launch_wave("cluster_extents", cn, ClusterExtents{ngen, d_rg_start.p, d_rg_len.p, d_list.p, d_v_first.p, layout_view(d_once.p), d_twice.p, d_owner.p, c0, 0});
                    int32_t* owner2 = (int32_t*)d_twice.p;
                    be.launch_wave("reader_mark", cn, ReaderMark{store_view(), d_v_row0.p, d_list2.p, ngen, d_rg_start.p, d_rg_len.p, d_list.p, d_v_first.p, layout_view(d_once.p), d_owner.p, owner2, c0, 1});
                    be.launch_wave("marker_look", cn, MarkerLook{store_view(), d_v_row0.p, d_list2.p, ngen, d_v_first.p, layout_view(d_once.p, false), d_owner.p, owner2, d_v_defer.p, c0});
                    be.launch_wave("reader_look", cn, ReaderLook{store_view(), d_v_row0.p, d_list2.p, ngen, d_rg_start.p, d_rg_len.p, d_list.p, d_v_first.p, d_lay_off.p, d_lay_bits.p, owner2, d_v_defer.p, c0});
                    be.launch_wave("reader_mark", cn, ReaderMark{store_view(), d_v_row0.p, d_list2.p, ngen, d_rg_start.p, d_rg_len.p, d_list.p, d_v_first.p, layout_view(d_once.p), d_owner.p, owner2, c0, 0});
                }
                defer = d_v_defer.p;
                exact_cluster_tests++;
            } else be.launch_wave("clusters_disjoint", ncl - 1, ClustersDisjoint{ngen, d_rg_start.p, d_rg_len.p, d_list.p, d_v_first.p, d_rg_count.p + 3, stage_first, force_unsure ? 1 : 0});
            be.launch_wave("cluster_validate", xcd_grid(na),
                           ClusterValidate{store_view(), layout_view(d_image.p), P, d_rg_start.p, d_rg_len.p, d_rg_info.p, d_rg_count.p, (uint64_t)cap,
                                           d_list.p, d_v_row0.p, d_list2.p, d_v_first.p, q, (uint32_t*)(d_rg_count.p + 1), na, 0, nullptr, d_rg_count.p + 3,
                                           d_foreign.p, d_foreign_count.p, (uint64_t)foreign_cap, d_foreign_masks.p, d_ms_key.p, generation_no, d_recwords.p, defer, d_v_done.p,
                                           d_rg_pkey.p, d_outw.p, d_outw_count.p, (uint64_t)kOutwCap});
            if (stage_first > 0) {
                be.launch("stage_gate", 1, StageGate{d_rg_count.p, (uint64_t)rg_count, force_gate ? 1 : 0});
                be.launch_wave("cluster_validate", xcd_grid(ncl - na),
                               ClusterValidate{store_view(), layout_view(d_image.p), P, d_rg_start.p, d_rg_len.p, d_rg_info.p, d_rg_count.p, (uint64_t)cap,
                                               d_list.p, d_v_row0.p, d_list2.p, d_v_first.p, q, (uint32_t*)(d_rg_count.p + 1), ncl - na, na, d_rg_count.p + 2, d_rg_count.p + 3,
                                               d_foreign.p, d_foreign_count.p, (uint64_t)foreign_cap, d_foreign_masks.p, d_ms_key.p, generation_no + 1, d_recwords.p, defer, d_v_done.p,
                                               d_rg_pkey.p, d_outw.p, d_outw_count.p, (uint64_t)kOutwCap});
            }
            be.launch_wave("outside_write_check", kOutwWaves,
                           OutsideWriteCheck{store_view(), d_rg_start.p, d_rg_len.p, d_rg_info.p, d_rg_pkey.p, d_rg_count.p, (uint64_t)cap, d_list.p, d_outw.p, d_outw_count.p, (uint64_t)kOutwCap,
                                             d_ms_key.p, anchor_table_rows, (uint32_t*)(d_rg_count.p + 1), kOutwWaves});
            if (info_count > 0) be.launch("store_info", info_count, StoreInfoOut{store_view(), info_first, d_rowinfo.p});
            be.mark(nullptr);
            group_downloads();
            if (info_count > 0) be.d2h_async(info, d_rowinfo.p, sizeof(RowInfo) * (size_t)info_count);
            be.d2h_async(&foreign_seen, d_foreign_count.p, 8);
            be.d2h_async(&outside_writes_call, d_outw_count.p, 8);
            be.d2h_async(done_h.data(), d_v_done.p, 4 * (size_t)ncl);
            be.d2h(head, d_rg_count.p, 32);
        };
        be.mark("validate");
        generation(clusters_out_of_order);
        if (head[3] != 0 && !clusters_out_of_order) {
            clusters_out_of_order = true;
            head[0] = (uint64_t)rg_count; head[1] = head[2] = head[3] = 0;
            be.mark("validate");
            generation(true);
        }
        *trouble = (uint32_t)head[1];
        outside_writes += (int64_t)outside_writes_call;
        const bool ran2 = stage_first > 0 && head[2] == 0;
        if (second_stage_ran) *second_stage_ran = ran2 ? 1 : 0;
        for (int64_t cl = 0; cl < ncl; cl++) {
            if (stage_first > 0 && cl >= na && !ran2) { done_h[(size_t)cl] = 0; continue; }
            const int64_t size = cluster_first[cl + 1] - cluster_first[cl];
            if (done_h[(size_t)cl] < size) {
                deferred_regions += size - done_h[(size_t)cl];
                if (!done && !*trouble) *trouble |= done_h[(size_t)cl] == 0 ? 8u : 1u;
            }
        }
        if (done) memcpy(done, done_h.data(), 4 * (size_t)ncl);
        if (head[0] > cap) { error = "region store overflow"; return -4; }
        const int64_t before = rg_count;
        rg_count = (int64_t)head[0];
        take_regions(before, rg_count, kids, kid_ids);
        collect_timing_more();
        return 0;
    }
    int store_judge(const int32_t* cur, const int32_t* back, int64_t n, int32_t d, int32_t* min_gap, int32_t* max_gap, uint8_t* verdict) {
        if (!resident) { error = "the session is not in resident mode"; return -2; }
        for (int64_t i = 0; i < n; i++) if (cur[i] < 0 || cur[i] >= ms_count || back[i] < 0 || back[i] >= ms_count) { error = "rows outside the MUM store"; return -2; }
        if (n == 0) return 0;
        begin_store_call();
        ensure(d_list, (size_t)n); ensure(d_list2, (size_t)n); ensure(d_j_min, (size_t)n); ensure(d_j_max, (size_t)n); ensure(d_small8, (size_t)n);
        int32_t* block = (int32_t*)be.staging(8 * (size_t)n);
        if (!block) { error = "cannot allocate the request staging block"; return -3; }
        memcpy(block, cur, 4 * (size_t)n); memcpy(block + n, back, 4 * (size_t)n);
        be.h2d_staged(d_list.p, block, 4 * (size_t)n); be.h2d_staged(d_list2.p, block + n, 4 * (size_t)n);
        be.mark("judge");
        be.launch_wave("judge_pairs", n, JudgePairs{store_view(), d_list.p, d_list2.p, d, d_j_min.p, d_j_max.p, d_small8.p});
        be.mark(nullptr);
        be.d2h_async(min_gap, d_j_min.p, 4 * (size_t)n); be.d2h_async(max_gap, d_j_max.p, 4 * (size_t)n);
        be.d2h(verdict, d_small8.p, (size_t)n);
        collect_timing_more();
        return 0;
    }
    int store_unmark(const int32_t* rows, int64_t n) {
        if (!resident || layout_rows < 0) { error = "the anchor list has not been settled"; return -2; }
        for (int64_t i = 0; i < n; i++) if (rows[i] < 0 || rows[i] >= ms_count) { error = "rows outside the MUM store"; return -2; }
        if (n == 0) return 0;
        ensure(d_list, (size_t)n);
        be.h2d(d_list.p, rows, 4 * (size_t)n);
        be.launch("store_unmark", n * ngen, StoreUnmark{store_view(), layout_view(d_image.p), d_list.p});
        return 0;
    }
    int store_fill(const int32_t* last_of, const int32_t* first_of_next, int64_t n, uint8_t* add, std::vector<int64_t>* starts, std::vector<int64_t>* ends) {
        if (!resident || layout_rows < 0) { error = "the anchor list has not been settled"; return -2; }
        for (int64_t i = 0; i < n; i++) if (last_of[i] < 0 || last_of[i] >= ms_count || first_of_next[i] < 0 || first_of_next[i] >= ms_count) { error = "rows outside the MUM store"; return -2; }
        starts->clear(); ends->clear();
        if (n == 0) return 0;
        begin_store_call();
        const size_t ngz = (size_t)ngen;
        ensure(d_list, (size_t)n); ensure(d_list2, (size_t)n); ensure(d_small8, (size_t)n); ensure(d_f_start, (size_t)n * ngz); ensure(d_f_end, (size_t)n * ngz);
        be.h2d(d_list.p, last_of, 4 * (size_t)n); be.h2d(d_list2.p, first_of_next, 4 * (size_t)n);
        be.mark("fill");
        be.launch_wave("fill_between", n, FillBetween{store_view(), layout_view(d_image.p, false), P, d_list.p, d_list2.p, d_small8.p, d_f_start.p, d_f_end.p});
        be.mark(nullptr);
        be.d2h(add, d_small8.p, (size_t)n);
        std::vector<int32_t> which;
        for (int64_t i = 0; i < n; i++) if (add[i] == 1) which.push_back((int32_t)i);
        if (!which.empty()) {
            const size_t m = which.size();
            ensure(d_list, m); ensure(d_f_pack, 2 * m * ngz);
            be.h2d(d_list.p, which.data(), 4 * m);
            be.launch("fill_gather", (int64_t)m * ngen, FillGather{d_list.p, ngen, d_f_start.p, d_f_end.p, d_f_pack.p});
            std::vector<int64_t> pack(2 * m * ngz);
            be.d2h(pack.data(), d_f_pack.p, 8 * pack.size());
            starts->resize(m * ngz); ends->resize(m * ngz);
            for (size_t k = 0; k < m; k++) {
                memcpy(starts->data() + k * ngz, pack.data() + (2 * k) * ngz, 8 * ngz);
                memcpy(ends->data() + k * ngz, pack.data() + (2 * k + 1) * ngz, 8 * ngz);
            }
        }
        collect_timing_more();
        return 0;
    }
    struct ChainInfo { int64_t n_in, lcbs_first, lcbs_dissolved, mums_dissolved, n_mums, n_lcbs, n_fillers; uint64_t trouble; };
    void order_check_launch(uint32_t* word, uint32_t bit) {
        const int64_t cnt = (int64_t)std::min<uint64_t>(foreign_seen, (uint64_t)foreign_cap);
        const int64_t rows = ms_count - layout_rows;
        if (cnt <= 0 || rows <= 0) return;
        ensure(d_hits, kHitCap); ensure(d_hit_count, 2); ensure(d_hit_owned, kHitCap * (size_t)ngen); ensure(d_hit_present, kHitCap * (size_t)ngen);
        be.memset(d_hit_count.p, 0, 16);
        const Store S = store_view();
        const Layout L = layout_view(d_image.p, false);
        be.launch_wave("foreign_bound", cnt, ForeignBound{S, L, P, d_rg_start.p, d_rg_len.p, d_foreign.p, cnt, d_foreign_masks.p, d_recwords.p, d_hits.p, d_hit_count.p, (uint64_t)kHitCap,
                                                         d_hit_owned.p, d_hit_present.p, word, bit});
        const int64_t chunks = (rows + kScanRows - 1) / kScanRows, waves = 8192;
        be.launch_wave("foreign_scan", waves, ForeignScan{S, d_rg_start.p, d_rg_len.p, d_ms_key.p, d_foreign.p, d_hits.p, d_hit_count.p, (uint64_t)kHitCap, d_hit_owned.p, d_hit_present.p,
                                                         layout_rows, ms_count, chunks, waves});
        be.launch_wave("foreign_decide_hits", (int64_t)kHitCap, ForeignDecideHits{S, L, P, d_rg_start.p, d_rg_len.p, d_foreign.p, d_foreign_masks.p, d_hits.p, d_hit_count.p, (uint64_t)kHitCap,
                                                                                 d_hit_owned.p, d_hit_present.p, word, bit});
        if (order_debug) {
            uint64_t nh = 0;
            be.d2h(&nh, d_hit_count.p, 8);
            fprintf(stderr, "[order check] %ld noted candidates, %ld left to the scan (launched for %ld), %ld recursion rows\n", (long)cnt, (long)nh, (long)kHitCap, (long)rows);
        }
    }
    int store_order_check(uint32_t* trouble) {
        if (!resident || layout_rows < 0) { error = "the anchor list has not been settled"; return -2; }
        *trouble = 0;
        begin_store_call();
        ensure(d_rg_count, 4);
        be.mark("validate");
        be.memset(d_rg_count.p + 1, 0, 8);
        order_check_launch((uint32_t*)(d_rg_count.p + 1), 1u);
        be.mark(nullptr);
        uint64_t word = 0;
        be.d2h(&word, d_rg_count.p + 1, 8);
        *trouble = (uint32_t)word;
        collect_timing_more();
        return 0;
    }
    int store_chain_begin(int64_t expect, int32_t d, float diag_diff, int64_t c) {
        if (!resident || layout_rows < 0) { error = "the anchor list has not been settled"; return -2; }
        if (expect <= 0 || expect > ms_count) { error = "bad MUM count"; return -2; }
        if (chain_event) { be.event_wait(chain_event); be.event_release(chain_event); chain_event = nullptr; }
        begin_store_call();
        const size_t rows = (size_t)ms_count, cap = (size_t)expect;
        ensure(d_ch_flag, rows + 1); ensure(d_ch_pos, rows + 1);
        ensure(d_ch_key, cap); ensure(d_ch_val, cap); ensure(d_ch_skey, cap); ensure(d_ch_srow, cap); ensure(d_ch_key2, cap); ensure(d_ch_row2, cap);
        ensure(d_ch_verdict, cap); ensure(d_ch_head, cap + 1); ensure(d_ch_hpos, cap + 1); ensure(d_ch_survive, cap + 1); ensure(d_ch_spos, cap + 1);
        ensure(d_ch_lcblen, cap); ensure(d_ch_hdr, kChWords); ensure(d_ch_outrow, cap); ensure(d_ch_outhead, cap);
        const size_t host_bytes = 8 * (size_t)kChWords + 4 * cap + cap;
        if (host_bytes > chain_host_cap) {
            if (chain_host) be.pinned_free(chain_host);
            chain_host_cap = 0;
            chain_host = (uint8_t*)be.pinned_alloc(host_bytes + host_bytes / 4 + 64);
            if (!chain_host) { error = "cannot allocate the chain result block"; return -3; }
            chain_host_cap = host_bytes + host_bytes / 4 + 64;
        }
        chain_cap = (int64_t)cap;
        const Store S = store_view();
        be.mark("chain");
        {
            const ClearJob jobs[] = {{d_ch_hdr.p, 8 * (size_t)kChWords, 0}, {d_ch_lcblen.p, 8 * cap, 0}};
            be.clear_many(jobs, 2);
        }
        order_check_launch((uint32_t*)(d_ch_hdr.p + kChTrouble), (uint32_t)kChainOrder);
        be.launch("chain_flag", (int64_t)rows + 1, ChainFlag{S, (int64_t)rows, d_ch_flag.p});
        be.exclusive_scan(d_ch_flag.p, d_ch_pos.p, rows + 1);
        be.launch("chain_keys", (int64_t)rows, ChainKeys{S, d_ch_pos.p, d_ch_key.p, d_ch_val.p, (int64_t)cap});
        be.sort_pairs(d_ch_key.p, d_ch_skey.p, d_ch_val.p, d_ch_srow.p, cap, bits_for((uint64_t)glen_h[0]));
        const int64_t* n1 = d_ch_pos.p + rows;
        int64_t* hdr = d_ch_hdr.p;
        uint64_t* trouble = (uint64_t*)(hdr + kChTrouble);
        const bool bp = diag_diff > 1.0f;
        int64_t* back = nullptr;
        if (bp) {
            ensure(d_ch_back, cap); ensure(d_ch_wflag, cap + 1); ensure(d_ch_wpos, cap + 1); ensure(d_ch_wend, cap); ensure(d_ch_wverdict, cap);
            ensure(d_ch_wlist, (size_t)kChainStarts); ensure(d_ch_wkeep, (size_t)kChainStarts);
            back = d_ch_back.p;
        }
        const int64_t nstarts = std::min<int64_t>((int64_t)cap, kChainStarts);
        auto windows = [&](const uint64_t* row, const int64_t* n) {
            be.launch("chain_starts", (int64_t)cap + 1, ChainHeads{d_ch_verdict.p, n, d_ch_wflag.p, kChPass});
            be.exclusive_scan(d_ch_wflag.p, d_ch_wpos.p, cap + 1);
            be.launch_wave("chain_window", (int64_t)cap, ChainWindow{S, row, n, d, diag_diff, d_ch_verdict.p, chain_window, d_ch_wpos.p, d_ch_wlist.p, d_ch_wend.p, d_ch_wverdict.p});
            be.launch("chain_select", 1, ChainSelect{n, d_ch_wpos.p, d_ch_wlist.p, d_ch_wend.p, d_ch_wkeep.p, trouble});
            be.launch_wave("chain_window_fill", nstarts, ChainWindowFill{n, d_ch_wpos.p, d_ch_wlist.p, d_ch_wend.p, d_ch_wverdict.p, d_ch_wkeep.p, trouble, d_ch_verdict.p, back});
        };
        be.launch_wave("chain_judge", (int64_t)cap, ChainJudge{S, d_ch_skey.p, d_ch_srow.p, n1, d, diag_diff, d_ch_verdict.p, trouble, force_chain_tie ? 1 : 0, back});
        be.launch("chain_judge_reverse", (int64_t)cap, ChainJudgeReverse{S, d_ch_srow.p, n1, d, diag_diff, d_ch_verdict.p});
        if (bp) windows(d_ch_srow.p, n1);
        be.launch("chain_heads", (int64_t)cap + 1, ChainHeads{d_ch_verdict.p, n1, d_ch_head.p, kChClose});
        be.exclusive_scan(d_ch_head.p, d_ch_hpos.p, cap + 1);
        be.launch("chain_lcb_sum", (int64_t)cap, ChainLcbSum{S, d_ch_srow.p, n1, d_ch_hpos.p, d_ch_verdict.p, d_ch_lcblen.p, hdr});
        be.launch("chain_dissolve", (int64_t)cap + 1, ChainDissolve{n1, d_ch_hpos.p, d_ch_head.p, d_ch_verdict.p, d_ch_lcblen.p, c, d_ch_survive.p, hdr});
        if (!bp) be.launch_wave("chain_unmark", (int64_t)cap, ChainUnmark{S, layout_view(d_image.p), d_ch_srow.p, n1, d_ch_survive.p, nullptr});
        be.exclusive_scan(d_ch_survive.p, d_ch_spos.p, cap + 1);
        be.launch("chain_compact", (int64_t)cap, ChainCompact{n1, d_ch_survive.p, d_ch_spos.p, d_ch_skey.p, d_ch_srow.p, d_ch_key2.p, d_ch_row2.p, hdr});
        const int64_t* n2 = hdr + kChN2;
        be.launch_wave("chain_judge", (int64_t)cap, ChainJudge{S, d_ch_key2.p, d_ch_row2.p, n2, d, diag_diff, d_ch_verdict.p, trouble, 0, back});
        be.launch("chain_judge_reverse", (int64_t)cap, ChainJudgeReverse{S, d_ch_row2.p, n2, d, diag_diff, d_ch_verdict.p});
        if (bp) {
            windows(d_ch_row2.p, n2);
            be.launch_wave("chain_unmark", (int64_t)cap, ChainUnmark{S, layout_view(d_image.p), d_ch_srow.p, n1, d_ch_survive.p, trouble});
        }
        be.launch("chain_heads", (int64_t)cap + 1, ChainHeads{d_ch_verdict.p, n2, d_ch_head.p, kChClose});
        be.exclusive_scan(d_ch_head.p, d_ch_hpos.p, cap + 1);
        if (cap > 1) be.launch_wave("chain_fill", (int64_t)cap - 1, ChainFill{S, layout_view(d_image.p, false), P, d_ch_row2.p, n2, d_ch_head.p, back, hdr});
        be.launch("chain_out", (int64_t)cap, ChainOut{d_ch_row2.p, n2, d_ch_head.p, d_ch_hpos.p, d_ch_verdict.p, d_ch_outrow.p, d_ch_outhead.p, hdr});
        be.mark(nullptr);
        be.d2h_async_pinned(chain_host, hdr, 8 * (size_t)kChWords);
        be.d2h_async_pinned(chain_host + 8 * (size_t)kChWords, d_ch_outrow.p, 4 * cap);
        be.d2h_async_pinned(chain_host + 8 * (size_t)kChWords + 4 * cap, d_ch_outhead.p, cap);
        chain_event = be.event_record();
        chain_pending = true;
        return 0;
    }
    int store_chain_end(ChainInfo* info, const int32_t** rows, const uint8_t** heads) {
        if (!chain_pending) { error = "no chain call in flight"; return -2; }
        chain_pending = false;
        if (chain_event) { be.event_wait(chain_event); be.event_release(chain_event); chain_event = nullptr; }
        else be.sync();
        const int64_t* h = (const int64_t*)chain_host;
        *info = ChainInfo{h[kChN1], h[kChLcb1], h[kChLcbDissolved], h[kChMumDissolved], h[kChN2], h[kChLcb2], h[kChFill], (uint64_t)h[kChTrouble]};
        *rows = (const int32_t*)(chain_host + 8 * (size_t)kChWords);
        *heads = chain_host + 8 * (size_t)kChWords + 4 * (size_t)chain_cap;
        collect_timing_more();
        chain_passed[0] = h[kChPass1]; chain_passed[1] = h[kChPass2];
        if (info->n_in != chain_cap) { error = "the MUM list of the caller and the accepted rows of the store differ"; return -2; }
        return 0;
    }
    int store_rows(const int32_t* rows, int64_t first, int64_t n, bool raw, int32_t* out_start, uint8_t* out_strand) {
        if (!resident) { error = "the session is not in resident mode"; return -2; }
        if (n == 0) return 0;
        const size_t ngz = (size_t)ngen;
        if (!rows) {
            if (first < 0 || first + n > ms_count) { error = "rows outside the MUM store"; return -2; }
            if (raw) {
                be.d2h_async(out_start, d_anchor_start.p + (size_t)first * ngz, 4 * (size_t)n * ngz);
                be.d2h(out_strand, d_ms_strand.p + (size_t)first * ngz, (size_t)n * ngz);
                return 0;
            }
        } else for (int64_t i = 0; i < n; i++) if (rows[i] < 0 || rows[i] >= ms_count) { error = "rows outside the MUM store"; return -2; }
        const int64_t piece = std::max<int64_t>(1, (int64_t)((32u << 20) / (5 * ngz)));
        ensure(d_list, (size_t)std::min(n, piece)); ensure(d_o_start, (size_t)std::min(n, piece) * ngz); ensure(d_o_strand, (size_t)std::min(n, piece) * ngz);
        std::vector<int32_t> seq;
        for (int64_t at = 0; at < n; at += piece) {
            const int64_t m = std::min(piece, n - at);
            const int32_t* src = rows ? rows + at : nullptr;
            if (!src) { seq.resize((size_t)m); for (int64_t i = 0; i < m; i++) seq[(size_t)i] = (int32_t)(first + at + i); src = seq.data(); }
            be.h2d(d_list.p, src, 4 * (size_t)m);
            be.launch("store_rows", m * ngen, StoreRowsOut{store_view(), d_list.p, d_o_start.p, d_o_strand.p, raw ? 1 : 0});
            be.d2h_async(out_start + (size_t)at * ngz, d_o_start.p, 4 * (size_t)m * ngz);
            be.d2h(out_strand + (size_t)at * ngz, d_o_strand.p, (size_t)m * ngz);
        }
        return 0;
    }
    int store_layout(uint64_t* out, int64_t words) {
        if (!resident || layout_rows < 0) { error = "the anchor list has not been settled"; return -2; }
        if ((size_t)words != layout_geometry()) { error = "layout size does not match"; return -2; }
        be.d2h(out, d_image.p, 8 * (size_t)words);
        return 0;
    }
    std::vector<int64_t> lay_off_h;

    int dense_build(const RegionInfo* R, int64_t nreg, int64_t nflag) {
        std::vector<int32_t> fi_h((size_t)nreg, -1), list_h;
        std::vector<int64_t> start_h(1, 0);
        for (int64_t r = 0; r < nreg; r++)
            if (dense_h[(size_t)r]) { fi_h[(size_t)r] = (int32_t)list_h.size(); list_h.push_back((int32_t)r); start_h.push_back(start_h.back() + R[r].nR); }
        const int64_t n = start_h.back();
        ensure(d_dfi, (size_t)nreg); ensure(d_dlist, (size_t)nflag); ensure(d_dstart, (size_t)nflag + 1);
        be.h2d(d_dfi.p, fi_h.data(), 4 * (size_t)nreg);
        be.h2d(d_dlist.p, list_h.data(), 4 * (size_t)nflag);
        be.h2d(d_dstart.p, start_h.data(), 8 * ((size_t)nflag + 1));
        ensure(d_dval2, (size_t)std::max<int64_t>(n, 1));
        dense_rounds = 0;
        if (n == 0) return 0;
        if (n >= (1ll << 31) || (uint64_t)nflag * 5 >= ((uint64_t)1 << 32)) { error = "suffix-array batch too large"; return -5; }
        ensure(d_dkey, (size_t)n); ensure(d_dval, (size_t)n); ensure(d_dkey2, (size_t)n);
        ensure(d_dhead, (size_t)n + 1); ensure(d_dfirst, (size_t)n + 1); ensure(d_dlcp, (size_t)n);
        DenseLevels L{};
        ensure(d_drank[0], (size_t)n);
        be.launch("dense_rank0", n, DenseRank0{P, d_R.p, d_dlist.p, d_dstart.p, nflag, d_drank[0].p});
        L.lv[0] = d_drank[0].p;
        int64_t groups = 0;
        int k = 0;
        for (; k + 1 < kDenseMaxLevels; k++) {
            const uint64_t top_rank = k == 0 ? (uint64_t)nflag * 5 : (uint64_t)n;
            be.launch("dense_keys", n, DenseKeys{d_dstart.p, nflag, d_drank[k].p, (int64_t)1 << k, d_dkey.p, d_dval.p});
            be.sort_pairs(d_dkey.p, d_dkey2.p, d_dval.p, d_dval2.p, (size_t)n, 32 + bits_for(top_rank));
            be.launch("dense_heads", n + 1, DenseHeads{d_dkey2.p, n, d_dhead.p});
            be.exclusive_scan(d_dhead.p, d_dfirst.p, (size_t)n + 1);
            ensure(d_drank[k + 1], (size_t)n);
            be.launch("dense_rerank", n, DenseRerank{d_dval2.p, d_dhead.p, d_dfirst.p, d_drank[k + 1].p});
            L.lv[k + 1] = d_drank[k + 1].p;
            be.d2h(&groups, d_dfirst.p + n, 8);
            if (groups == n) break;
        }
        if (groups != n) { error = "suffix-array sort did not converge"; return -5; }
        dense_rounds = k + 1;
        L.top = k;
        be.launch("dense_lcp", n, DenseLcp{L, d_dval2.p, d_dstart.p, nflag, d_dlcp.p});
        be.launch("dense_rep", n, DenseRep{d_R.p, d_dlist.p, d_dval2.p, d_dstart.p, nflag, d_dlcp.p, d_rep.p});
        return 0;
    }
    bool dense_mode = false;
    std::vector<uint8_t> dense_h;
    void collect_timing_more() { for (const PhaseTime& t : be.collect()) timing.push_back(t); }

    int allgather_host(const void* send, int64_t bytes, void* recv) {
        if (!coll.device) return coll.allgather(coll.ctx, send, bytes, recv);
        ensure(d_hsend, (size_t)bytes); ensure(d_hrecv, (size_t)bytes * (size_t)coll.world);
        be.h2d(d_hsend.p, send, (size_t)bytes);
        if (be.allgather_dev(d_hsend.p, bytes, d_hrecv.p)) return 1;
        be.d2h(recv, d_hrecv.p, (size_t)bytes * (size_t)coll.world);
        return 0;
    }

    std::vector<uint64_t> ev_key_h, ev_val_h;
    std::vector<int32_t> rep_h;
    int ev_lbits = 0;
    int64_t work_budget = 1 << 22;
    int64_t dirty_min = 4096;
    int64_t flagged_div = 8;
    int64_t tangled_max = 1 << 17;
    bool fast_tail = true;
    int64_t tail_repeats = 0;
    bool tangle_rounds = true;
    bool group_small = true;
    bool group_wide = false;
    int64_t last_grouped = 0;
    int64_t last_grouped_wide = 0, last_handed_back = -1, last_wide_regions = 0;
    bool force_atomic_marks = false;
    int filter_factor = 8;
    int slot_factor = 2;
    bool bucket_sort = true;
    bool index_build = true;
    int64_t index_bucket_min = 1 << 24;
    bool index_verify = false;
    int64_t index_overflow_cap = 0;
    int64_t last_index_bucketed = 0, last_index_overflow = 0, last_index_lost = -1;
    bool master_seg = true;
    bool force_gate = false;
    int64_t chain_window = 4096;
    int64_t chain_passed[2] = {-1, -1};
    bool force_chain_tie = false;
    bool force_unsure = false;
    bool order_debug = false;
    int64_t outside_writes = 0;
    int64_t exact_cluster_tests = 0;
    int64_t deferred_regions = 0;
    bool clusters_out_of_order = false;
    int64_t hint_shrink = 1;
    bool phase_timing = true;
    bool tune(const std::string& key, int64_t value) {
        if (key == "flagged_div" && value >= 1) { flagged_div = value; return true; }
        if (key == "tangled_max" && value >= 0) { tangled_max = value; return true; }
        if (key == "tangle_rounds") { tangle_rounds = value != 0; return true; }
        if (key == "fast_tail") { fast_tail = value != 0; return true; }
        if (key == "atomic_marks") { force_atomic_marks = value != 0; return true; }
        if (key == "master_seg") { master_seg = value != 0; return true; }
        if (key == "bucket_sort") { bucket_sort = value != 0; return true; }
        if (key == "index_build") { index_build = value != 0; return true; }
        if (key == "index_bucket_min" && value >= 1) { index_bucket_min = value; return true; }
        if (key == "index_verify") { index_verify = value != 0; return true; }
        if (key == "index_overflow_cap" && value >= 0) { index_overflow_cap = value; return true; }
        if (key == "filter_factor") { filter_factor = value < 1 ? 1 : (int)value; return true; }
        if (key == "slot_factor") { slot_factor = value < 1 ? 1 : (int)value; return true; }
        if (key == "stage_gate") { force_gate = value != 0; return true; }
        if (key == "chain_window" && value >= 1 && value <= kChainWindowMax) { chain_window = value; return true; }
        if (key == "chain_tie") { force_chain_tie = value != 0; return true; }
        if (key == "cluster_unsure") { force_unsure = value != 0; return true; }
        if (key == "order_debug") { order_debug = value != 0; return true; }
        if (key == "timing") { phase_timing = value != 0; be.timing_on = phase_timing; return true; }
        if (key == "group_small") { group_small = value != 0; return true; }
        if (key == "group_wide") { group_wide = value != 0; return true; }
        if (key == "work_budget" && value > 0) { work_budget = value; return true; }
        if (key == "dense_all") { dense_all = value != 0; return true; }
        if (key == "dirty_min" && value >= 0) { dirty_min = value; return true; }
        if (key == "hint_shrink" && value >= 1) { hint_shrink = value; return true; }
        if (key == "copy_kernel") { return tune_copy_kernel(be, value != 0, 0); }
        return false;
    }

    void release() {
        if (chain_event) { be.event_wait(chain_event); be.event_release(chain_event); chain_event = nullptr; }
        for (BufBase* b : all_bufs) { if (b->raw) be.free(b->raw); b->raw = nullptr; b->cap = 0; }
        if (chain_host) be.pinned_free(chain_host);
        chain_host = nullptr; chain_host_cap = 0; chain_pending = false;
        if (blk) be.free(blk);
        if (d_goff) be.free(d_goff);
        if (d_glen) be.free(d_glen);
        blk = nullptr; d_goff = nullptr; d_glen = nullptr;
    }

    struct DeviceOutOfMemory { size_t bytes; };

private:
    B& be;
    struct BufBase { void* raw = nullptr; size_t cap = 0; };
    std::vector<BufBase*> all_bufs;
    template <class T> struct Buf : BufBase {
        T* p = nullptr;
    };
    template <class T> void ensure(Buf<T>& b, size_t n) {
        if (n <= b.cap && b.p) return;
        if (std::find(all_bufs.begin(), all_bufs.end(), (BufBase*)&b) == all_bufs.end()) all_bufs.push_back(&b);
        if (b.raw) be.free(b.raw);
        b.raw = nullptr; b.p = nullptr; b.cap = 0;
        const size_t want = n + n / 4 + 16;
        b.raw = be.alloc(want * sizeof(T));
        if (!b.raw) throw DeviceOutOfMemory{want * sizeof(T)};
        b.p = (T*)b.raw; b.cap = want;
    }
    template <class T> void ensure_keep(Buf<T>& b, size_t n, size_t keep) {
        if (n <= b.cap && b.p) return;
        if (std::find(all_bufs.begin(), all_bufs.end(), (BufBase*)&b) == all_bufs.end()) all_bufs.push_back(&b);
        const size_t want = n + n / 2 + 16;
        void* raw = be.alloc(want * sizeof(T));
        if (!raw) throw DeviceOutOfMemory{want * sizeof(T)};
        if (b.p && keep) { be.d2d(raw, b.p, keep * sizeof(T)); be.sync(); }
        if (b.raw) be.free(b.raw);
        b.raw = raw; b.p = (T*)raw; b.cap = want;
    }
    void collect_timing() { timing = be.collect(); }
    template <class T> static auto group_on(T& b, int) -> decltype(b.d2h_group(), void()) { b.d2h_group(); }
    template <class T> static void group_on(T&, long) {}
    template <class T> static auto flush_on(T& b, int) -> decltype(b.d2h_flush(), void()) { b.d2h_flush(); }
    template <class T> static void flush_on(T&, long) {}
    template <class T> static auto tune_copy_kernel(T& b, bool on, int) -> decltype(b.group_copies = on, true) { b.group_copies = on; return true; }
    template <class T> static bool tune_copy_kernel(T&, bool, long) { return true; }
    template <class T> static auto sort_keys_on(T& b, uint64_t* ki, uint64_t* ko, size_t n, int lo, int hi, int) -> decltype(b.sort_keys(ki, ko, n, lo, hi), true) { b.sort_keys(ki, ko, n, lo, hi); return true; }
    template <class T> static bool sort_keys_on(T&, uint64_t*, uint64_t*, size_t, int, int, long) { return false; }
    void group_downloads() { group_on(be, 0); }
    void flush_downloads() { flush_on(be, 0); }

    SeqBlock* blk = nullptr; int64_t* d_goff = nullptr; int64_t* d_glen = nullptr;
    int64_t total_words = 0;
    Packed P{};
    size_t ev_cap_hint = 0, cand_cap_hint = 0, rest_cap_hint[2] = {0, 0}, grp_cap_hint = 0;
    struct CallHint { int64_t units = 0, ncand = 0, nok = 0; };
    std::vector<CallHint> call_hints;
    int64_t call_ordinal = 0;
    Buf<uint8_t> d_gflag; Buf<int64_t> d_glo;
    Buf<int64_t> d_bkbase, d_bkbegin, d_ovf; Buf<uint64_t> d_ikey, d_ikey2, d_ikey3, d_ikey4;
    Buf<RegionInfo> d_R; Buf<int64_t> d_starts, d_lens, d_posbase;
    Buf<uint64_t> d_slots; Buf<uint32_t> d_filter, d_repeated; Buf<int32_t> d_next, d_rep, d_run, d_epm;
    Buf<int64_t> d_ucount, d_uoff; Buf<UnitRec> d_units;
    Buf<uint64_t> d_counter, d_evkey, d_evval, d_evkey2, d_evval2, d_evkey3, d_evval3; Buf<int64_t> d_sliceoff;
    Buf<int64_t> d_lo, d_cov; Buf<EventAtK> d_state; Buf<PairState> d_wsummary; Buf<int32_t> d_emax;
    Buf<uint64_t> d_cand; Buf<GenomeAtK> d_at; Buf<uint8_t> d_ok; Buf<int32_t> d_ok_k, d_ok_lon, d_osp; Buf<uint8_t> d_ofwd;
    Buf<uint64_t> d_wmask; Buf<int64_t> d_wcount, d_woff;
    Buf<int64_t> d_bcount, d_bbegin, d_pbase;
    Buf<int64_t> d_okcnt, d_okpos, d_cbase; Buf<int32_t> d_coarse; Buf<int32_t> d_creg, d_ck, d_clon, d_csp; Buf<uint8_t> d_cfwd;
    Buf<uint32_t> d_cflags, d_dirty; Buf<int32_t> d_bmax, d_bmin;
    Buf<GenomeAtK> d_xsend, d_xrecv; Buf<uint8_t> d_hsend, d_hrecv;
    Buf<RestItem> d_rest; Buf<uint64_t> d_qcount;
    Buf<uint8_t> d_dense; Buf<int32_t> d_dfi, d_dlist, d_dlcp; Buf<int64_t> d_dstart, d_dhead, d_dfirst;
    Buf<uint64_t> d_dkey, d_dkey2, d_dval, d_dval2; Buf<uint32_t> d_drank[kDenseMaxLevels];
    Buf<int32_t> d_anchor_start, d_anchor_lon; Buf<uint32_t> d_anchor_flags;
    int64_t table_counter = 0;
    Buf<uint64_t> d_image;
    Buf<uint8_t> d_ms_strand, d_ms_state, d_small8, d_o_strand; Buf<int32_t> d_ms_shift, d_ms_len, d_list, d_list2, d_j_min, d_j_max, d_o_start;
    Buf<int64_t> d_rg_start, d_rg_len, d_lay_off, d_lay_bits, d_v_row0, d_v_first, d_f_start, d_f_end, d_f_pack; Buf<RegInfo> d_rg_info; Buf<uint64_t> d_rg_count, d_once, d_twice;
    Buf<RowInfo> d_rowinfo; Buf<uint64_t> d_alg;
    Buf<int64_t> d_sd_cnt, d_sd_off; Buf<uint8_t> d_sd_keep;
    Buf<uint64_t> d_t_rem; Buf<uint8_t> d_t_done;
    Buf<int32_t> d_v_done, d_owner; Buf<uint8_t> d_v_defer, d_v_involved;
    Buf<uint64_t> d_t_left; uint64_t tangle_left[8] = {0, 0, 0, 0, 0, 0, 0, 0}; int tangle_ran = 0;
    Buf<int64_t> d_rg_pkey; Buf<OutsideWrite> d_outw; Buf<uint64_t> d_outw_count; int64_t rg_pkey_init = 0; uint64_t outside_writes_call = 0;
    Buf<ForeignRead> d_foreign; Buf<uint64_t> d_foreign_count, d_foreign_masks; Buf<int64_t> d_ms_key;
    size_t foreign_cap = 0; int64_t ms_key_rows = 0; uint64_t foreign_seen = 0;
    static constexpr size_t kHitCap = 256;
    Buf<uint64_t> d_hit_count, d_hit_owned, d_hit_present; Buf<int32_t> d_hits; Buf<uint8_t> d_recwords;
    Buf<int64_t> d_ch_flag, d_ch_pos, d_ch_head, d_ch_hpos, d_ch_survive, d_ch_spos, d_ch_hdr;
    Buf<uint64_t> d_ch_key, d_ch_val, d_ch_skey, d_ch_srow, d_ch_key2, d_ch_row2, d_ch_lcblen;
    Buf<uint8_t> d_ch_verdict, d_ch_outhead; Buf<int32_t> d_ch_outrow;
    Buf<int64_t> d_ch_back, d_ch_wflag, d_ch_wpos, d_ch_wlist, d_ch_wend; Buf<uint8_t> d_ch_wverdict, d_ch_wkeep;
    uint8_t* chain_host = nullptr; size_t chain_host_cap = 0; void* chain_event = nullptr; bool chain_pending = false; int64_t chain_cap = 0;
    size_t lay_words = 0, rg_cap_hint = 0;
    int64_t layout_rows = -1;
};

}
```

### parsnp_amd/csrc/engine/engine_hip.hip

```cpp
#include <cstdlib>
#include <cstring>
#include <dlfcn.h>
#include <unistd.h>
#include <hip/hip_runtime.h>
#include <rccl/rccl.h>
#include <rocprim/rocprim.hpp>

#include <atomic>
#include <chrono>
#include <map>
#include <string>
#include <thread>
#include <vector>

#include "engine_core.h"

namespace {

template <class F>
__global__ __launch_bounds__(256) void pm_kernel(F f, int64_t n) {
    int64_t tid = (int64_t)blockIdx.x * 256 + threadIdx.x;
    if (tid < n) f(tid);
}

__global__ __launch_bounds__(256) void pm_fill16(uint4* p, uint4 v, int64_t n16) {
    const int64_t per = 16 * 256;
    int64_t i = (int64_t)blockIdx.x * per + threadIdx.x;
#pragma unroll
    for (int k = 0; k < 16; k++, i += 256) if (i < n16) p[i] = v;
}

struct FillJobs { enum { kMax = 12 }; void* p[kMax]; unsigned long long bytes[kMax]; unsigned int value[kMax]; unsigned int first_block[kMax + 1]; int n; };
__global__ __launch_bounds__(256) void pm_fill_many(FillJobs jobs) {
    int j = 0;
    while (j + 1 < jobs.n && blockIdx.x >= jobs.first_block[j + 1]) j++;
    const unsigned long long off = (unsigned long long)(blockIdx.x - jobs.first_block[j]) << 16;
    const unsigned long long n = jobs.bytes[j];
    unsigned char* base = (unsigned char*)jobs.p[j];
    const unsigned int w = jobs.value[j];
    if ((((uintptr_t)base) & 15) == 0) {
        uint4* q = (uint4*)(base + off);
        const unsigned long long n16 = (n > off ? (n - off < 65536 ? n - off : 65536) : 0) >> 4;
#pragma unroll
        for (int k = 0; k < 16; k++) { const unsigned long long i = (unsigned long long)k * 256 + threadIdx.x; if (i < n16) q[i] = make_uint4(w, w, w, w); }
        for (unsigned long long i = off + (n16 << 4) + threadIdx.x; i < n && i < off + 65536; i += 256) base[i] = (unsigned char)w;
    } else {
        for (unsigned long long i = off + threadIdx.x; i < n && i < off + 65536; i += 256) base[i] = (unsigned char)w;
    }
}

struct CopyJobs { enum { kMax = 12 }; const void* src[kMax]; void* dst[kMax]; unsigned long long bytes[kMax]; unsigned int first_block[kMax + 1]; int n; };
__global__ __launch_bounds__(256) void pm_copy_many(CopyJobs jobs) {
    int j = 0;
    while (j + 1 < jobs.n && blockIdx.x >= jobs.first_block[j + 1]) j++;
    const unsigned long long off = (unsigned long long)(blockIdx.x - jobs.first_block[j]) << 16;
    const unsigned long long n = jobs.bytes[j];
    if (off >= n) return;
    const unsigned long long len = n - off < 65536 ? n - off : 65536;
    const unsigned char* s = (const unsigned char*)jobs.src[j] + off;
    unsigned char* d = (unsigned char*)jobs.dst[j] + off;
    unsigned long long done = 0;
    if ((((uintptr_t)s) & 15) == 0) {
        const unsigned long long n16 = len >> 4;
        for (unsigned long long i = threadIdx.x; i < n16; i += 256) ((uint4*)d)[i] = ((const uint4*)s)[i];
        done = n16 << 4;
    } else if ((((uintptr_t)s) & 3) == 0) {
        const unsigned long long n4 = len >> 2;
        for (unsigned long long i = threadIdx.x; i < n4; i += 256) ((unsigned int*)d)[i] = ((const unsigned int*)s)[i];
        done = n4 << 2;
    }
    for (unsigned long long i = done + threadIdx.x; i < len; i += 256) d[i] = s[i];
}

template <class F>
__global__ __launch_bounds__(64) void pm_wave_kernel(F f, int64_t n) {
    const int64_t w = (int64_t)blockIdx.x;
    if (w < n) f.wave(w);
}

struct Rccl {
    void* lib = nullptr;
    ncclResult_t (*GetUniqueId)(ncclUniqueId*) = nullptr;
    ncclResult_t (*CommInitRank)(ncclComm_t*, int, ncclUniqueId, int) = nullptr;
    ncclResult_t (*AllReduce)(const void*, void*, size_t, ncclDataType_t, ncclRedOp_t, ncclComm_t, hipStream_t) = nullptr;
    ncclResult_t (*AllGather)(const void*, void*, size_t, ncclDataType_t, ncclComm_t, hipStream_t) = nullptr;
    ncclResult_t (*CommDestroy)(ncclComm_t) = nullptr;
    ncclResult_t (*CommCount)(const ncclComm_t, int*) = nullptr;
    const char* (*GetErrorString)(ncclResult_t) = nullptr;
    std::string err;
    static Rccl& get() {
        static Rccl r;
        if (r.lib || !r.err.empty()) return r;
        const char* path = getenv("PARSNP_RCCL_LIB");
        if (!path || !*path) path = "/opt/rocm/lib/librccl.so.1";
        r.lib = dlopen(path, RTLD_NOW | RTLD_LOCAL);
        if (!r.lib) { r.err = std::string("cannot load RCCL (") + path + "): " + dlerror(); return r; }
        auto sym = [&](const char* n) { void* p = dlsym(r.lib, n); if (!p && r.err.empty()) r.err = std::string("RCCL symbol missing: ") + n; return p; };
        r.GetUniqueId = (decltype(r.GetUniqueId))sym("ncclGetUniqueId");
        r.CommInitRank = (decltype(r.CommInitRank))sym("ncclCommInitRank");
        r.AllReduce = (decltype(r.AllReduce))sym("ncclAllReduce");
        r.AllGather = (decltype(r.AllGather))sym("ncclAllGather");
        r.CommDestroy = (decltype(r.CommDestroy))sym("ncclCommDestroy");
        r.CommCount = (decltype(r.CommCount))sym("ncclCommCount");
        r.GetErrorString = (decltype(r.GetErrorString))sym("ncclGetErrorString");
        return r;
    }
    bool ok() const { return lib && err.empty(); }
};

struct HipBackend {
    hipStream_t stream = nullptr;
    int device = 0;
    void bind() { check(hipSetDevice(device), "hipSetDevice"); }
    void bind_thread() { bind(); }
    ncclComm_t comm = nullptr;
    std::string err;
    void* tmp = nullptr;
    size_t tmp_cap = 0;
    std::vector<std::pair<const char*, hipEvent_t>> marks;
    std::vector<hipEvent_t> pool;

    bool check(hipError_t e, const char* what) {
        if (e == hipSuccess) return true;
        if (err.empty()) err = std::string(what) + ": " + hipGetErrorString(e);
        return false;
    }
    bool ok() const { return err.empty(); }
    std::string error() const { return err; }

    ~HipBackend() {
        for (auto& m : marks) pool.push_back(m.second);
        for (auto e : pool) (void)hipEventDestroy(e);
        if (tmp) (void)hipFree(tmp);
        if (stage_p) (void)hipHostFree(stage_p);
        if (ring) (void)hipHostFree(ring);
        if (dring) (void)hipHostFree(dring);
        if (comm) (void)Rccl::get().CommDestroy(comm);
        if (stream) (void)hipStreamDestroy(stream);
    }
    bool nccl_check(ncclResult_t r, const char* what) {
        if (r == ncclSuccess) return true;
        if (err.empty()) err = std::string(what) + ": " + Rccl::get().GetErrorString(r);
        return false;
    }
    bool comm_init(int rank, int world, const uint8_t* id128) {
        Rccl& R = Rccl::get();
        if (!R.ok()) { if (err.empty()) err = R.err; return false; }
        ncclUniqueId id;
        static_assert(sizeof(ncclUniqueId) == 128, "PM_RCCL_ID_BYTES");
        memcpy(&id, id128, sizeof id);
        const int limit = getenv("PARSNP_RCCL_TIMEOUT") ? atoi(getenv("PARSNP_RCCL_TIMEOUT")) : 180;
        std::atomic<bool> done{false};
        std::thread dog;
        if (limit > 0)
            dog = std::thread([&done, limit, rank, world] {
                for (int t = 0; t < limit * 10 && !done.load(); t++) std::this_thread::sleep_for(std::chrono::milliseconds(100));
                if (!done.load()) {
                    fprintf(stderr, "parsnp engine: rank %d of %d: the RCCL communicator did not come up within %d s (ranks with different ids? a rank that never started?)\n", rank, world, limit);
                    _exit(4);
                }
            });
        const ncclResult_t r = R.CommInitRank(&comm, world, id, rank);
        done.store(true);
        if (dog.joinable()) dog.join();
        return nccl_check(r, "ncclCommInitRank");
    }
    int comm_ranks() { int n = 0; if (comm && Rccl::get().CommCount(comm, &n) == ncclSuccess) return n; return 0; }
    void fill32(int32_t* p, int32_t v) { check(hipMemsetD32Async((hipDeviceptr_t)p, v, 1, stream), "hipMemsetD32Async"); }
    int allreduce_min_i32_dev(int32_t* d, int64_t count) {
        if (!comm) { if (err.empty()) err = "no RCCL communicator"; return 1; }
        return nccl_check(Rccl::get().AllReduce(d, d, (size_t)count, ncclInt32, ncclMin, comm, stream), "ncclAllReduce(min)") ? 0 : 1;
    }
    int allgather_dev(const void* send, int64_t bytes, void* recv) {
        if (!comm) { if (err.empty()) err = "no RCCL communicator"; return 1; }
        return nccl_check(Rccl::get().AllGather(send, recv, (size_t)bytes, ncclUint8, comm, stream), "ncclAllGather") ? 0 : 1;
    }
    void* alloc(size_t n) { void* p = nullptr; if (!check(hipMalloc(&p, n ? n : 1), "hipMalloc")) return nullptr; return p; }
    void free(void* p) { check(hipFree(p), "hipFree"); }
    static void* host_alloc(size_t n) { return malloc(n ? n : 1); }
    static void host_free(void* p) { ::free(p); }
    void memset(void* p, int v, size_t n) {
        if (n >= ((size_t)1 << 20) && ((uintptr_t)p & 15) == 0) {
            const int64_t n16 = (int64_t)(n >> 4);
            const uint32_t w = 0x01010101u * (uint32_t)(uint8_t)v;
            hipLaunchKernelGGL(pm_fill16, dim3((unsigned)((n16 + 4095) / 4096)), dim3(256), 0, stream, (uint4*)p, make_uint4(w, w, w, w), n16);
            check(hipGetLastError(), "pm_fill16");
            const size_t done = (size_t)n16 << 4;
            if (done < n) check(hipMemsetAsync((char*)p + done, v, n - done, stream), "hipMemsetAsync");
            return;
        }
        check(hipMemsetAsync(p, v, n, stream), "hipMemsetAsync");
    }
    void clear_many(const pm::ClearJob* jobs, int n) {
        FillJobs f; f.n = 0; unsigned int blocks = 0;
        for (int i = 0; i < n; i++) {
            if (!jobs[i].bytes) continue;
            if (f.n == FillJobs::kMax) { launch_fill(f, blocks); f.n = 0; blocks = 0; }
            f.p[f.n] = jobs[i].p; f.bytes[f.n] = jobs[i].bytes; f.value[f.n] = 0x01010101u * (unsigned int)(uint8_t)jobs[i].value; f.first_block[f.n] = blocks;
            blocks += (unsigned int)((jobs[i].bytes + 65535) >> 16);
            f.n++;
        }
        if (f.n) launch_fill(f, blocks);
    }
    void launch_fill(FillJobs& f, unsigned int blocks) {
        f.first_block[f.n] = blocks;
        hipLaunchKernelGGL(pm_fill_many, dim3(blocks), dim3(256), 0, stream, f);
        check(hipGetLastError(), "pm_fill_many");
    }
    std::atomic<uint64_t> bytes_h2d{0}, bytes_d2h{0};
    static bool copy_log() { static const bool on = getenv("PARSNP_COPY_LOG") != nullptr; return on; }
    static double now_us() { return std::chrono::duration<double, std::micro>(std::chrono::steady_clock::now().time_since_epoch()).count(); }
    uint8_t* ring = nullptr; size_t ring_at = 0; static constexpr size_t kRing = (size_t)4 << 20;
    void h2d(void* d, const void* s, size_t n) {
        const double t0 = copy_log() ? now_us() : 0;
        bytes_h2d += n;
        if (n && n <= kRing / 4) {
            if (!ring && hipHostMalloc((void**)&ring, kRing, hipHostMallocDefault) != hipSuccess) ring = nullptr;
            if (ring) {
                const size_t need = (n + 63) & ~(size_t)63;
                if (ring_at + need > kRing) { check(hipStreamSynchronize(stream), "sync"); ring_at = 0; }
                memcpy(ring + ring_at, s, n);
                check(hipMemcpyAsync(d, ring + ring_at, n, hipMemcpyHostToDevice, stream), "hipMemcpy H2D (ring)");
                ring_at += need;
                if (copy_log()) fprintf(stderr, "[copy] h2d (ring) %8zu B %8.1f us\n", n, now_us() - t0);
                return;
            }
        }
        if (n) check(hipMemcpyAsync(d, s, n, hipMemcpyHostToDevice, stream), "hipMemcpy H2D"); check(hipStreamSynchronize(stream), "sync");
        if (copy_log()) fprintf(stderr, "[copy] h2d       %9zu B %8.1f us\n", n, now_us() - t0);
    }
    uint8_t* dring = nullptr; size_t dring_at = 0; static constexpr size_t kDRing = (size_t)48 << 20;
    struct Landing { void* dst; const uint8_t* at; size_t n; };
    std::vector<Landing> landings;
    void land() { for (const Landing& l : landings) memcpy(l.dst, l.at, l.n); landings.clear(); dring_at = 0; }
    void drop_landings() { group.n = 0; group_blocks = 0; grouping = false; if (!landings.empty()) { (void)hipStreamSynchronize(stream); landings.clear(); dring_at = 0; } }
    bool group_copies = true;
    bool grouping = false; CopyJobs group{}; unsigned int group_blocks = 0; uint8_t* dring_dev = nullptr;
    static constexpr size_t kGroupMax = (size_t)4 << 20;
    void d2h_group() { if (group_copies) grouping = true; }
    void d2h_flush() { flush_group(); }
    void flush_group() {
        if (group.n) {
            group.first_block[group.n] = group_blocks;
            hipLaunchKernelGGL(pm_copy_many, dim3(group_blocks), dim3(256), 0, stream, group);
            check(hipGetLastError(), "pm_copy_many");
            group.n = 0; group_blocks = 0;
        }
    }
    void d2h_async(void* d, const void* s, size_t n) {
        const double t0 = copy_log() ? now_us() : 0;
        bytes_d2h += n;
        if (!n) return;
        const size_t need = (n + 255) & ~(size_t)255;
        if (!dring && hipHostMalloc((void**)&dring, kDRing, hipHostMallocDefault) != hipSuccess) dring = nullptr;
        if (grouping && dring && !dring_dev) {
            void* dp = nullptr;
            if (hipHostGetDevicePointer(&dp, dring, 0) == hipSuccess && dp) dring_dev = (uint8_t*)dp; else { (void)hipGetLastError(); group_copies = false; grouping = false; }
        }
        if (grouping && dring && n <= kGroupMax && dring_at + need <= kDRing) {
            if (group.n == CopyJobs::kMax) flush_group();
            group.src[group.n] = s; group.dst[group.n] = dring_dev + dring_at; group.bytes[group.n] = n; group.first_block[group.n] = group_blocks;
            group_blocks += (unsigned int)((n + 65535) >> 16);
            group.n++;
            landings.push_back(Landing{d, dring + dring_at, n});
            dring_at += need;
            if (copy_log()) fprintf(stderr, "[copy] d2h_group %9zu B\n", n);
            return;
        }
        if (dring && dring_at + need <= kDRing) {
            check(hipMemcpyAsync(dring + dring_at, s, n, hipMemcpyDeviceToHost, stream), "hipMemcpy D2H (ring)");
            landings.push_back(Landing{d, dring + dring_at, n});
            dring_at += need;
        } else check(hipMemcpyAsync(d, s, n, hipMemcpyDeviceToHost, stream), "hipMemcpy D2H");
        if (copy_log()) fprintf(stderr, "[copy] d2h_async %9zu B %8.1f us\n", n, now_us() - t0);
    }
    void d2h_async_pinned(void* d, const void* s, size_t n) {
        bytes_d2h += n; if (n) check(hipMemcpyAsync(d, s, n, hipMemcpyDeviceToHost, stream), "hipMemcpy D2H (pinned)");
    }
    void d2h(void* d, const void* s, size_t n) {
        const double t0 = copy_log() ? now_us() : 0;
        d2h_async(d, s, n); sync();
        if (copy_log()) fprintf(stderr, "[copy] d2h       %9zu B %8.1f us (with the queued work before it)\n", n, now_us() - t0);
    }
    void sync() { flush_group(); grouping = false; check(hipStreamSynchronize(stream), "hipStreamSynchronize"); land(); }
    void* event_record() {
        hipEvent_t e = nullptr;
        if (!pool.empty()) { e = pool.back(); pool.pop_back(); }
        else if (!check(hipEventCreate(&e), "hipEventCreate")) return nullptr;
        check(hipEventRecord(e, stream), "hipEventRecord");
        return (void*)e;
    }
    static void event_wait(void* e) { if (e) (void)hipEventSynchronize((hipEvent_t)e); }
    void event_release(void* e) { if (e) pool.push_back((hipEvent_t)e); }
    void* stage_p = nullptr; size_t stage_cap = 0;
    void* staging(size_t n) {
        if (n > stage_cap) {
            if (stage_p) (void)hipHostFree(stage_p);
            stage_p = nullptr; stage_cap = 0;
            if (!check(hipHostMalloc(&stage_p, n + n / 4 + 4096, hipHostMallocDefault), "hipHostMalloc(staging)")) return nullptr;
            stage_cap = n + n / 4 + 4096;
        }
        return stage_p;
    }
    void d2d(void* d, const void* s, size_t n) { if (n) check(hipMemcpyAsync(d, s, n, hipMemcpyDeviceToDevice, stream), "hipMemcpy D2D"); }
    void* pinned_alloc(size_t n) { void* p = nullptr; if (!check(hipHostMalloc(&p, n ? n : 1, hipHostMallocDefault), "hipHostMalloc")) return nullptr; return p; }
    void pinned_free(void* p) { if (p) (void)hipHostFree(p); }
    void h2d_staged(void* d, const void* s, size_t n) {
        bytes_h2d += n; if (n) check(hipMemcpyAsync(d, s, n, hipMemcpyHostToDevice, stream), "hipMemcpy H2D (staged)");
        if (getenv("PARSNP_COPY_LOG")) fprintf(stderr, "[copy] h2d_staged %8zu B\n", n);
    }

    static int upload_threads() { const char* e = getenv("PARSNP_UPLOAD_THREADS"); const int v = e ? atoi(e) : 0; return v >= 1 && v <= 32 ? v : 4; }
    bool stage_genomes(int n, const uint8_t* const* seqs, const int64_t* lens, const std::vector<char>& take, const std::vector<int64_t>& goff,
                       pm::SeqBlock* blk, int64_t maxlen) {
        int64_t total = 0;
        for (int g = 0; g < n; g++) if (take[(size_t)g]) total += lens[g];
        const int kThreads = total < (8 << 20) ? 1 : upload_threads();
        constexpr int kPer = 2;
        int device = 0;
        if (!check(hipGetDevice(&device), "hipGetDevice")) return false;
        check(hipStreamSynchronize(stream), "sync");
        struct Slot { uint8_t* host = nullptr; uint8_t* dev = nullptr; hipStream_t st = nullptr; hipEvent_t done = nullptr; bool used = false; };
        std::vector<Slot> slots((size_t)kThreads * kPer);
        bool ok = true;
        const size_t cap = (size_t)std::max<int64_t>(maxlen, 1);
        for (auto& sl : slots)
            ok = ok && hipHostMalloc((void**)&sl.host, cap, hipHostMallocDefault) == hipSuccess && hipMalloc((void**)&sl.dev, cap) == hipSuccess &&
                 hipStreamCreateWithFlags(&sl.st, hipStreamNonBlocking) == hipSuccess && hipEventCreateWithFlags(&sl.done, hipEventDisableTiming) == hipSuccess;
        std::vector<int> failed((size_t)kThreads, 0);
        if (ok) {
            auto work = [&](int t) {
                if (hipSetDevice(device) != hipSuccess) { failed[(size_t)t] = 1; return; }
                int turn = 0;
                for (int g = t; g < n; g += kThreads) {
                    if (!take[(size_t)g]) continue;
                    Slot& sl = slots[(size_t)t * kPer + (size_t)(turn++ % kPer)];
                    if (sl.used && hipEventSynchronize(sl.done) != hipSuccess) { failed[(size_t)t] = 1; return; }
                    memcpy(sl.host, seqs[g], (size_t)lens[g]);
                    bytes_h2d += (uint64_t)lens[g];
                    if (hipMemcpyAsync(sl.dev, sl.host, (size_t)lens[g], hipMemcpyHostToDevice, sl.st) != hipSuccess) { failed[(size_t)t] = 1; return; }
                    const int64_t nblk = (lens[g] + 31) / 32;
                    for (int s = 0; s < 2; s++)
                        hipLaunchKernelGGL(pm_kernel<pm::PackStrand>, dim3((unsigned)((nblk + 255) / 256)), dim3(256), 0, sl.st,
                                           pm::PackStrand{sl.dev, lens[g], s, blk, goff[2 * (size_t)g + (size_t)s] / 32}, nblk);
                    if (hipGetLastError() != hipSuccess || hipEventRecord(sl.done, sl.st) != hipSuccess) { failed[(size_t)t] = 1; return; }
                    sl.used = true;
                }
            };
            std::vector<std::thread> th;
            for (int t = 1; t < kThreads; t++) th.emplace_back(work, t);
            work(0);
            for (auto& x : th) x.join();
        }
        for (auto& sl : slots) {
            if (sl.st) { if (hipStreamSynchronize(sl.st) != hipSuccess) ok = false; (void)hipStreamDestroy(sl.st); }
            if (sl.done) (void)hipEventDestroy(sl.done);
            if (sl.host) (void)hipHostFree(sl.host);
            if (sl.dev) (void)hipFree(sl.dev);
        }
        for (int f : failed) if (f) ok = false;
        if (!ok && err.empty()) err = "staging the genomes failed (allocation, copy or PackStrand launch)";
        return ok;
    }

    template <class F> void launch(const char* name, int64_t n, F f) {
        if (n <= 0) return;
        int64_t blocks = (n + 255) / 256;
        if (blocks > 0x7fffffffll) { if (err.empty()) err = std::string("grid too large: ") + name; return; }
        hipLaunchKernelGGL(pm_kernel<F>, dim3((unsigned)blocks), dim3(256), 0, stream, f, n);
        check(hipGetLastError(), name);
    }
    template <class F> void launch_wave(const char* name, int64_t n, F f) {
        if (n <= 0) return;
        if (n > 0x7fffffffll) { if (err.empty()) err = std::string("grid too large: ") + name; return; }
        hipLaunchKernelGGL(pm_wave_kernel<F>, dim3((unsigned)n), dim3(64), 0, stream, f, n);
        check(hipGetLastError(), name);
    }
    void need_tmp(size_t n) {
        if (n <= tmp_cap) return;
        if (tmp) (void)hipFree(tmp);
        tmp = nullptr; tmp_cap = 0;
        if (check(hipMalloc(&tmp, n + n / 4 + 256), "hipMalloc(tmp)")) tmp_cap = n + n / 4 + 256;
    }
    void exclusive_scan(const int64_t* in, int64_t* out, size_t n) {
        size_t bytes = 0;
        check(rocprim::exclusive_scan(nullptr, bytes, in, out, (int64_t)0, n, rocprim::plus<int64_t>(), stream), "scan size");
        need_tmp(bytes);
        check(rocprim::exclusive_scan(tmp, bytes, in, out, (int64_t)0, n, rocprim::plus<int64_t>(), stream), "exclusive_scan");
    }
    void sort_pairs(uint64_t* ki, uint64_t* ko, uint64_t* vi, uint64_t* vo, size_t n, int bits) {
        size_t bytes = 0;
        check(rocprim::radix_sort_pairs(nullptr, bytes, ki, ko, vi, vo, n, 0, (unsigned)bits, stream), "sort size");
        need_tmp(bytes);
        check(rocprim::radix_sort_pairs(tmp, bytes, ki, ko, vi, vo, n, 0, (unsigned)bits, stream), "radix_sort_pairs");
    }

    void sort_keys(uint64_t* ki, uint64_t* ko, size_t n, int begin_bit, int end_bit) {
        size_t bytes = 0;
        check(rocprim::radix_sort_keys(nullptr, bytes, ki, ko, n, (unsigned)begin_bit, (unsigned)end_bit, stream), "sort size");
        need_tmp(bytes);
        check(rocprim::radix_sort_keys(tmp, bytes, ki, ko, n, (unsigned)begin_bit, (unsigned)end_bit, stream), "radix_sort_keys");
    }

    bool timing_on = true;
    void mark(const char* name) {
        if (!timing_on) return;
        hipEvent_t e;
        if (!pool.empty()) { e = pool.back(); pool.pop_back(); }
        else if (!check(hipEventCreate(&e), "hipEventCreate")) return;
        check(hipEventRecord(e, stream), "hipEventRecord");
        marks.emplace_back(name, e);
    }
    std::vector<pm::PhaseTime> collect() {
        std::vector<pm::PhaseTime> out;
        sync();
        for (size_t i = 0; i + 1 < marks.size(); i++) {
            if (!marks[i].first) continue;
            float ms = 0;
            check(hipEventElapsedTime(&ms, marks[i].second, marks[i + 1].second), "hipEventElapsedTime");
            bool merged = false;
            for (auto& t : out) if (!strcmp(t.name, marks[i].first)) { t.ms += ms; merged = true; }
            if (!merged) out.push_back(pm::PhaseTime{marks[i].first, ms});
        }
        for (auto& m : marks) pool.push_back(m.second);
        marks.clear();
        return out;
    }
};

}

typedef HipBackend PmBackend;
static const char* pm_backend_name = "hip";
static PmBackend* pm_backend_open(int device, std::string* err) {
    int count = 0;
    hipError_t e = hipGetDeviceCount(&count);
    if (e != hipSuccess || count == 0) {
        *err = std::string("no HIP device available (") + (e == hipSuccess ? "0 devices" : hipGetErrorString(e)) + "); this engine has no CPU path";
        return nullptr;
    }
    if (device < 0) {
        const char* e = getenv("PARSNP_DEVICE");
        if (e && *e) device = atoi(e);
    }
    if (device >= 0) {
        if (device >= count || hipSetDevice(device) != hipSuccess) { *err = "cannot select the requested HIP device"; return nullptr; }
    }
    HipBackend* b = new HipBackend;
    (void)hipGetDevice(&b->device);
    if (hipStreamCreateWithFlags(&b->stream, hipStreamNonBlocking) != hipSuccess) { *err = "hipStreamCreate failed"; delete b; return nullptr; }
    return b;
}
#define PM_HAVE_RCCL 1
#include "abi_glue.h"
```

Before: 31180.

## Batch small fills and copies into one kernel and defer tangle readback

Adds a batch queue that collects small memsets, device-to-device copies, pinned downloads and table uploads into one multi-job kernel launch. The queue is flushed before any other stream command, which cuts per-call launch and memcpy overhead on the host. Also folds the qcount clear and the settle setup clears into existing clear_many calls, and moves the tangle_left readback to later download points. The cost is added complexity around flushing before frees and syncs, with a risk of ordering bugs.

```diff
diff --git a/parsnp_amd/csrc/engine/batch.h b/parsnp_amd/csrc/engine/batch.h
--- /dev/null
+++ b/parsnp_amd/csrc/engine/batch.h
@@ -0,0 +1,132 @@
+#pragma once
+#include <cstddef>
+#include <cstdint>
+
+#if defined(__HIPCC__)
+#define PM_BATCH_HD __host__ __device__
+#else
+#define PM_BATCH_HD
+#endif
+
+namespace pm {
+
+struct BatchTable {
+    enum { kMax = 24 };
+    void* dst[kMax];
+    const void* src[kMax];
+    unsigned long long bytes[kMax];
+    unsigned int value[kMax];
+    unsigned int first_block[kMax + 1];
+    int n;
+};
+
+constexpr unsigned int kBatchPieceShift = 16;
+constexpr unsigned int kBatchThreads = 256;
+
+struct Batch {
+    BatchTable t;
+    unsigned int blocks = 0;
+    Batch() { t.n = 0; }
+    bool empty() const { return t.n == 0; }
+    void clear() { t.n = 0; blocks = 0; }
+    static bool overlap(const void* a, size_t an, const void* b, size_t bn) {
+        const uintptr_t x = (uintptr_t)a, y = (uintptr_t)b;
+        return an && bn && x < y + bn && y < x + an;
+    }
+    bool conflicts(const void* dst, const void* src, size_t bytes) const {
+        for (int j = 0; j < t.n; j++) {
+            const size_t m = (size_t)t.bytes[j];
+            if (overlap(dst, bytes, t.dst[j], m)) return true;
+            if (t.src[j] && overlap(dst, bytes, t.src[j], m)) return true;
+            if (src && overlap(src, bytes, t.dst[j], m)) return true;
+        }
+        return false;
+    }
+    bool add(void* dst, const void* src, size_t bytes, unsigned int value) {
+        if (!bytes) return true;
+        const unsigned long long nb = ((unsigned long long)bytes + ((1ull << kBatchPieceShift) - 1)) >> kBatchPieceShift;
+        if (t.n == BatchTable::kMax || (unsigned long long)blocks + nb > 0x7fffffffull || conflicts(dst, src, bytes)) return false;
+        t.dst[t.n] = dst; t.src[t.n] = src; t.bytes[t.n] = bytes; t.value[t.n] = value; t.first_block[t.n] = blocks;
+        blocks += (unsigned int)nb;
+        t.n++;
+        return true;
+    }
+    bool add_fill(void* p, size_t bytes, int byte_value) { return add(p, nullptr, bytes, 0x01010101u * (unsigned int)(uint8_t)byte_value); }
+    bool add_copy(void* dst, const void* src, size_t bytes) { return add(dst, src, bytes, 0); }
+    const BatchTable& close() { t.first_block[t.n] = blocks; return t; }
+};
+
+struct BatchVec16 { unsigned int x, y, z, w; };
+
+PM_BATCH_HD inline void batch_thread(const BatchTable& t, unsigned int block, unsigned int tid) {
+    int j = 0;
+    while (j + 1 < t.n && block >= t.first_block[j + 1]) j++;
+    const unsigned long long off = (unsigned long long)(block - t.first_block[j]) << kBatchPieceShift;
+    const unsigned long long n = t.bytes[j];
+    if (off >= n) return;
+    const unsigned long long len = n - off < (1ull << kBatchPieceShift) ? n - off : (1ull << kBatchPieceShift);
+    unsigned char* d = (unsigned char*)t.dst[j] + off;
+    if (!t.src[j]) {
+        const unsigned int w = t.value[j];
+        unsigned long long head = (16 - ((uintptr_t)d & 15)) & 15;
+        if (head > len) head = len;
+        if (tid < head) d[tid] = (unsigned char)w;
+        const unsigned long long n16 = (len - head) >> 4;
+        BatchVec16* q = (BatchVec16*)(d + head);
+        const BatchVec16 v = {w, w, w, w};
+#pragma unroll 4
+        for (unsigned long long i = tid; i < n16; i += kBatchThreads) q[i] = v;
+        const unsigned long long done = head + (n16 << 4);
+        if (done + tid < len) d[done + tid] = (unsigned char)w;
+        return;
+    }
+    const unsigned char* s = (const unsigned char*)t.src[j] + off;
+    const unsigned int skew = (unsigned int)(((uintptr_t)d - (uintptr_t)s) & 15);
+    if (skew == 0) {
+        unsigned long long head = (16 - ((uintptr_t)d & 15)) & 15;
+        if (head > len) head = len;
+        if (tid < head) d[tid] = s[tid];
+        const unsigned long long n16 = (len - head) >> 4;
+        BatchVec16* q = (BatchVec16*)(d + head);
+        const BatchVec16* r = (const BatchVec16*)(s + head);
+#pragma unroll 4
+        for (unsigned long long i = tid; i < n16; i += kBatchThreads) q[i] = r[i];
+        const unsigned long long done = head + (n16 << 4);
+        if (done + tid < len) d[done + tid] = s[done + tid];
+    } else if ((skew & 3) == 0) {
+        unsigned long long head = (4 - ((uintptr_t)d & 3)) & 3;
+        if (head > len) head = len;
+        if (tid < head) d[tid] = s[tid];
+        const unsigned long long n4 = (len - head) >> 2;
+        unsigned int* q = (unsigned int*)(d + head);
+        const unsigned int* r = (const unsigned int*)(s + head);
+#pragma unroll 4
+        for (unsigned long long i = tid; i < n4; i += kBatchThreads) q[i] = r[i];
+        const unsigned long long done = head + (n4 << 2);
+        if (done + tid < len) d[done + tid] = s[done + tid];
+    } else {
+        for (unsigned long long i = tid; i < len; i += kBatchThreads) d[i] = s[i];
+    }
+}
+
+template <class X> struct BatchQueue {
+    X* x = nullptr;
+    Batch b;
+    size_t upload_max = 0;
+    void flush() { if (!b.empty()) { const unsigned int blocks = b.blocks; x->batch_run(b.close(), blocks); b.clear(); } }
+    void drop() { b.clear(); }
+    void fill(void* p, size_t bytes, int byte_value) {
+        if (!b.add_fill(p, bytes, byte_value)) { flush(); (void)b.add_fill(p, bytes, byte_value); }
+    }
+    void copy(void* dst, const void* src, size_t bytes) {
+        if (!b.add_copy(dst, src, bytes)) { flush(); (void)b.add_copy(dst, src, bytes); }
+    }
+    void upload(void* dst, const void* src_dev, const void* src_host, size_t bytes) {
+        if (!bytes) return;
+        if (bytes <= upload_max) { copy(dst, src_dev, bytes); return; }
+        flush();
+        x->upload_command(dst, src_host, bytes);
+    }
+};
+
+}
diff --git a/parsnp_amd/csrc/engine/engine_core.h b/parsnp_amd/csrc/engine/engine_core.h
--- a/parsnp_amd/csrc/engine/engine_core.h
+++ b/parsnp_amd/csrc/engine/engine_core.h
@@ -352,12 +352,13 @@
         ensure(d_wmask, (size_t)nwv + 1); ensure(d_wcount, (size_t)nwv + 1); ensure(d_woff, (size_t)nwv + 1);
         if (from_store_) ensure(d_alg, 8 * (size_t)kAlgSets);
         ensure(d_dense, regz);
+        ensure(d_qcount, (size_t)kSlices * kSliceStride);
         {
             const ClearJob jobs[] = {
                 {d_filter.p, sizeof(uint32_t) * (size_t)fwords_clear, 0}, {d_slots.p, sizeof(uint64_t) * (size_t)tsize_clear, 0xff}, {d_counter.p, 8 * ncounter, 0},
                 {d_repeated.p, 4 * (size_t)(npos / 32 + 2), 0}, {d_coarse.p, 4 * (size_t)std::max<int64_t>(centries, 1), 0},
                 {d_ucount.p + npairs, 8, 0}, {d_wcount.p + nwv, 8, 0}, {from_store_ ? d_alg.p : nullptr, from_store_ ? (size_t)64 * kAlgSets : 0, 0},
-                {dense_mode ? nullptr : d_dense.p, dense_mode ? 0 : regz, 0}};
+                {dense_mode ? nullptr : d_dense.p, dense_mode ? 0 : regz, 0}, {d_qcount.p, 8 * (size_t)kSlices * kSliceStride, 0}};
             be.clear_many(jobs, (int)(sizeof jobs / sizeof jobs[0]));
         }
         int64_t nflag = 0;
@@ -461,7 +462,7 @@
                                    GroupedPairEventsWide{P, d_R.p, d_starts.p, d_lens.p, ngen, d_rep.p, d_evkey3.p, d_evval3.p, d_counter.p + kGrpSlot, (uint64_t)grp_cap, lbits,
                                                          d_glo.p, g_first, g_last, d_gflag.p, d_state.p, d_emax.p, d_epm.p, (int64_t)nreg, first_form ? 1 : 0, d_counter.p + kWideSlot});
             }
-            be.memset(d_qcount.p, 0, 8 * (size_t)kSlices * kSliceStride);
+            if (again) be.memset(d_qcount.p, 0, 8 * (size_t)kSlices * kSliceStride);
             be.mark("seed_extend");
             be.launch("seed_extend", nunits * 64,
                       SeedExtend{P, d_R.p, d_units.p, d_slots.p, d_filter.p, d_next.p, d_rep.p, d_repeated.p,
@@ -836,6 +837,7 @@
     int settle_launch(int64_t table_id) {
         if (int rc = need_resident(table_id)) return rc;
         begin_store_call();
+        tangle_fetch = 0;
         const int64_t rows = anchor_table_rows;
         const size_t words = layout_geometry();
         ensure(d_image, words);
@@ -846,30 +848,37 @@
         be.memset(d_image.p, 0, 8 * words);
         ensure(d_recwords, words);
         be.memset(d_recwords.p, 0, words);
+        ensure(d_sd_cnt, (size_t)rows + 1);
+        be.memset(d_sd_cnt.p + rows, 0, 8);
         const Store S = store_view();
         const Layout L = layout_view(d_image.p);
         be.launch_wave("settle_clean", rows, SettleClean{S, P});
-        std::vector<int32_t> fl;
-        for (int64_t c = 0; c < rows; c++) { const uint32_t f = anchor_flags_h[(size_t)c]; if (!(f & (kRowBad | kRowOutside)) && (f & kRowDirty)) fl.push_back((int32_t)c); }
+        std::vector<int32_t>& fl = settle_flagged_h;
+        fl.clear();
+        if (fl.capacity() < (size_t)rows) fl.reserve((size_t)rows);
+        bool ordered = true;
+        for (int64_t c = 0; c < rows; c++) {
+            const uint32_t f = anchor_flags_h[(size_t)c];
+            if (!(f & (kRowBad | kRowOutside)) && (f & kRowDirty)) fl.push_back((int32_t)c);
+            if ((f & kRowEarly) && !(f & (kRowBad | kRowOutside | kRowDirty))) ordered = false;
+        }
+        if (!fl.empty()) {
+            const uint64_t* before_once = d_once.p; const uint64_t* before_twice = d_twice.p;
+            ensure(d_once, words); ensure(d_twice, words); ensure(d_list, fl.size());
+            ensure(d_t_rem, 2); ensure(d_t_done, fl.size());
+            if (d_once.p != before_once || d_twice.p != before_twice) { be.memset(d_once.p, 0, 8 * words); be.memset(d_twice.p, 0, 8 * words); }
+            be.h2d(d_list.p, fl.data(), 4 * fl.size());
+            const ClearJob jobs[] = {{d_t_rem.p, 16, 0}, {d_t_done.p, fl.size(), 0}};
+            be.clear_many(jobs, 2);
+        }
         const bool many_flagged = flagged_div > 1 && fl.size() * (size_t)flagged_div > (size_t)rows;
-        bool ordered = true;
-        for (int64_t c = 0; c < rows && ordered; c++) { const uint32_t f = anchor_flags_h[(size_t)c]; ordered = !((f & kRowEarly) && !(f & (kRowBad | kRowOutside | kRowDirty))); }
         if (ordered && !force_atomic_marks) be.launch_wave("store_mark_ordered", ((rows + kMarkRows - 1) / kMarkRows) * ((ngen + 63) / 64), StoreMarkOrdered{S, L, rows});
         else be.launch("store_mark", rows * ngen, StoreMark{S, L, 0, (uint8_t)(kStAccepted | kStFlagged), kStAccepted});
         be.launch("layout_sentinel", (int64_t)ngen, LayoutSentinel{d_lay_off.p, d_lay_bits.p, d_image.p});
         if (!fl.empty()) {
-            const uint64_t* before_once = d_once.p; const uint64_t* before_twice = d_twice.p;
-            ensure(d_once, words); ensure(d_twice, words); ensure(d_list, fl.size());
-            if (d_once.p != before_once || d_twice.p != before_twice) { be.memset(d_once.p, 0, 8 * words); be.memset(d_twice.p, 0, 8 * words); }
-            be.h2d(d_list.p, fl.data(), 4 * fl.size());
             be.launch("collide_mark", (int64_t)fl.size() * ngen, CollideMark{S, d_list.p, layout_view(d_once.p), d_twice.p});
             be.launch_wave("collide_test", (int64_t)fl.size(), CollideTest{S, d_list.p, layout_view(d_twice.p, false)});
             be.launch("collide_clear", (int64_t)fl.size() * ngen, CollideClear{S, d_list.p, layout_view(d_once.p), d_twice.p});
-            ensure(d_t_rem, 2); ensure(d_t_done, fl.size());
-            {
-                const ClearJob jobs[] = {{d_t_rem.p, 16, 0}, {d_t_done.p, fl.size(), 0}};
-                be.clear_many(jobs, 2);
-            }
             be.launch("count_tangled", (int64_t)fl.size(), CountTangled{S, d_list.p, d_t_rem.p});
             if (many_flagged) {
                 uint64_t tangled = 0;
@@ -899,12 +908,14 @@
                 be.launch_wave("tangle_settle", (int64_t)fl.size(), TangleSettle{S, layout_view(d_image.p, false), P, d_list.p, d_owner.p, d_t_done.p, d_t_rem.p});
                 be.launch_wave("tangle_clear", (int64_t)fl.size(), TangleClear{S, d_list.p, d_lay_off.p, d_lay_bits.p, d_owner.p, d_t_done.p, d_t_rem.p, d_t_left.p + round});
             }
-            tangle_ran = 0;
-            if (rounds) { be.d2h_async(tangle_left, d_t_left.p, 8 * (size_t)rounds); tangle_ran = rounds; }
             be.launch_wave("settle_tangled", 1, SettleTangled{S, L, P, d_list.p, (int64_t)fl.size(), d_t_done.p, d_t_rem.p});
+            tangle_ran = 0; tangle_fetch = rounds;
         }
         layout_rows = rows;
         return 0;
+    }
+    void fetch_tangle_left() {
+        if (tangle_fetch) { be.d2h_async(tangle_left, d_t_left.p, 8 * (size_t)tangle_fetch); tangle_ran = tangle_fetch; tangle_fetch = 0; }
     }
     int store_settle_seeds(int64_t table_id, int32_t q, RowInfo* out, std::vector<RegInfo>* infos, std::vector<int32_t>* ids) {
         infos->clear(); ids->clear();
@@ -923,7 +934,6 @@
         be.launch("anchor_list", rows, AnchorList{S, d_ch_pos.p, d_list.p});
         const int64_t* nacc = d_ch_pos.p + rows;
         const Layout L = layout_view(d_image.p, false);
-        be.memset(d_sd_cnt.p + rows, 0, 8);
         be.launch_wave("seed_count", xcd_grid(rows), SeedCount{S, L, P, d_list.p, nacc, q, d_sd_cnt.p, d_sd_keep.p, rows});
         be.exclusive_scan(d_sd_cnt.p, d_sd_off.p, (size_t)rows + 1);
         size_t cap = std::max<size_t>(rg_cap_hint, (size_t)rows / 4 + 1024);
@@ -937,6 +947,7 @@
             group_downloads();
             if (guess) be.d2h_async(raw.data(), d_rg_info.p, sizeof(RegInfo) * guess);
             if (!again) be.d2h_async(out, d_rowinfo.p, sizeof(RowInfo) * (size_t)rows);
+            fetch_tangle_left();
             int64_t got = 0;
             be.d2h(&got, d_sd_off.p + rows, 8);
             if ((size_t)got <= cap) {
@@ -965,6 +976,7 @@
         ensure(d_rowinfo, (size_t)count);
         be.launch("store_info", count, StoreInfoOut{store_view(), first, d_rowinfo.p});
         be.mark(nullptr);
+        fetch_tangle_left();
         be.d2h(out, d_rowinfo.p, sizeof(RowInfo) * (size_t)count);
         collect_timing_more();
         return 0;
@@ -1501,6 +1513,7 @@
         if (key == "dirty_min" && value >= 0) { dirty_min = value; return true; }
         if (key == "hint_shrink" && value >= 1) { hint_shrink = value; return true; }
         if (key == "copy_kernel") { return tune_copy_kernel(be, value != 0, 0); }
+        if (key == "batch_small") { return tune_batch(be, value != 0, 0); }
         return false;
     }
 
@@ -1551,6 +1564,8 @@
     template <class T> static void flush_on(T&, long) {}
     template <class T> static auto tune_copy_kernel(T& b, bool on, int) -> decltype(b.group_copies = on, true) { b.group_copies = on; return true; }
     template <class T> static bool tune_copy_kernel(T&, bool, long) { return true; }
+    template <class T> static auto tune_batch(T& b, bool on, int) -> decltype(b.set_batch(on)) { return b.set_batch(on); }
+    template <class T> static bool tune_batch(T&, bool, long) { return true; }
     template <class T> static auto sort_keys_on(T& b, uint64_t* ki, uint64_t* ko, size_t n, int lo, int hi, int) -> decltype(b.sort_keys(ki, ko, n, lo, hi), true) { b.sort_keys(ki, ko, n, lo, hi); return true; }
     template <class T> static bool sort_keys_on(T&, uint64_t*, uint64_t*, size_t, int, int, long) { return false; }
     void group_downloads() { group_on(be, 0); }
@@ -1577,6 +1592,7 @@
     Buf<uint32_t> d_cflags, d_dirty; Buf<int32_t> d_bmax, d_bmin;
     Buf<GenomeAtK> d_xsend, d_xrecv; Buf<uint8_t> d_hsend, d_hrecv;
     Buf<RestItem> d_rest; Buf<uint64_t> d_qcount;
+    std::vector<int32_t> settle_flagged_h;
     Buf<uint8_t> d_dense; Buf<int32_t> d_dfi, d_dlist, d_dlcp; Buf<int64_t> d_dstart, d_dhead, d_dfirst;
     Buf<uint64_t> d_dkey, d_dkey2, d_dval, d_dval2; Buf<uint32_t> d_drank[kDenseMaxLevels];
     Buf<int32_t> d_anchor_start, d_anchor_lon; Buf<uint32_t> d_anchor_flags;
@@ -1588,7 +1604,7 @@
     Buf<int64_t> d_sd_cnt, d_sd_off; Buf<uint8_t> d_sd_keep;
     Buf<uint64_t> d_t_rem; Buf<uint8_t> d_t_done;
     Buf<int32_t> d_v_done, d_owner; Buf<uint8_t> d_v_defer, d_v_involved;
-    Buf<uint64_t> d_t_left; uint64_t tangle_left[8] = {0, 0, 0, 0, 0, 0, 0, 0}; int tangle_ran = 0;
+    Buf<uint64_t> d_t_left; uint64_t tangle_left[8] = {0, 0, 0, 0, 0, 0, 0, 0}; int tangle_ran = 0, tangle_fetch = 0;
     Buf<int64_t> d_rg_pkey; Buf<OutsideWrite> d_outw; Buf<uint64_t> d_outw_count; int64_t rg_pkey_init = 0; uint64_t outside_writes_call = 0;
     Buf<ForeignRead> d_foreign; Buf<uint64_t> d_foreign_count, d_foreign_masks; Buf<int64_t> d_ms_key;
     size_t foreign_cap = 0; int64_t ms_key_rows = 0; uint64_t foreign_seen = 0;
diff --git a/parsnp_amd/csrc/engine/engine_hip.hip b/parsnp_amd/csrc/engine/engine_hip.hip
--- a/parsnp_amd/csrc/engine/engine_hip.hip
+++ b/parsnp_amd/csrc/engine/engine_hip.hip
@@ -14,6 +14,7 @@
 #include <vector>
 
 #include "engine_core.h"
+#include "batch.h"
 
 namespace {
 
@@ -71,6 +72,8 @@
     }
     for (unsigned long long i = done + threadIdx.x; i < len; i += 256) d[i] = s[i];
 }
+
+__global__ __launch_bounds__(256) void pm_batch(pm::BatchTable t) { pm::batch_thread(t, blockIdx.x, threadIdx.x); }
 
 template <class F>
 __global__ __launch_bounds__(64) void pm_wave_kernel(F f, int64_t n) {
@@ -120,6 +123,7 @@
     std::vector<std::pair<const char*, hipEvent_t>> marks;
     std::vector<hipEvent_t> pool;
 
+    HipBackend() { bq.x = this; bq.upload_max = kUploadKernelMax; }
     bool check(hipError_t e, const char* what) {
         if (e == hipSuccess) return true;
         if (err.empty()) err = std::string(what) + ": " + hipGetErrorString(e);
@@ -166,20 +170,49 @@
         return nccl_check(r, "ncclCommInitRank");
     }
     int comm_ranks() { int n = 0; if (comm && Rccl::get().CommCount(comm, &n) == ncclSuccess) return n; return 0; }
-    void fill32(int32_t* p, int32_t v) { check(hipMemsetD32Async((hipDeviceptr_t)p, v, 1, stream), "hipMemsetD32Async"); }
+    void fill32(int32_t* p, int32_t v) { about_to_enqueue(); check(hipMemsetD32Async((hipDeviceptr_t)p, v, 1, stream), "hipMemsetD32Async"); }
     int allreduce_min_i32_dev(int32_t* d, int64_t count) {
         if (!comm) { if (err.empty()) err = "no RCCL communicator"; return 1; }
+        about_to_enqueue();
         return nccl_check(Rccl::get().AllReduce(d, d, (size_t)count, ncclInt32, ncclMin, comm, stream), "ncclAllReduce(min)") ? 0 : 1;
     }
     int allgather_dev(const void* send, int64_t bytes, void* recv) {
         if (!comm) { if (err.empty()) err = "no RCCL communicator"; return 1; }
+        about_to_enqueue();
         return nccl_check(Rccl::get().AllGather(send, recv, (size_t)bytes, ncclUint8, comm, stream), "ncclAllGather") ? 0 : 1;
     }
     void* alloc(size_t n) { void* p = nullptr; if (!check(hipMalloc(&p, n ? n : 1), "hipMalloc")) return nullptr; return p; }
-    void free(void* p) { check(hipFree(p), "hipFree"); }
+    void free(void* p) { if (!bq.b.empty()) { bind(); about_to_enqueue(); } check(hipFree(p), "hipFree"); }
     static void* host_alloc(size_t n) { return malloc(n ? n : 1); }
     static void host_free(void* p) { ::free(p); }
+    bool batch_on = true;
+    pm::BatchQueue<HipBackend> bq;
+    static constexpr size_t kUploadKernelMax = (size_t)1 << 20;
+    uint64_t batch_launches = 0, batch_jobs = 0;
+    void batch_run(const pm::BatchTable& t, unsigned int blocks) {
+        batch_launches++; batch_jobs += (uint64_t)t.n;
+        if (copy_log()) fprintf(stderr, "[copy] pm_batch  %d jobs, %u workgroups\n", t.n, blocks);
+        hipLaunchKernelGGL(pm_batch, dim3(blocks), dim3(256), 0, stream, t);
+        check(hipGetLastError(), "pm_batch");
+    }
+    void upload_command(void* d, const void* s, size_t n) { check(hipMemcpyAsync(d, s, n, hipMemcpyHostToDevice, stream), "hipMemcpy H2D"); }
+    void about_to_enqueue() { bq.flush(); }
+    bool set_batch(bool on) { about_to_enqueue(); flush_group(); batch_on = on; return true; }
+    static void* device_view(void* host) {
+        void* dp = nullptr;
+        if (hipHostGetDevicePointer(&dp, host, 0) == hipSuccess && dp) return dp;
+        (void)hipGetLastError();
+        return nullptr;
+    }
+    struct PinnedView { const uint8_t* host = nullptr; uint8_t* dev = nullptr; size_t bytes = 0; };
+    PinnedView stage_view, pinned_view;
+    void* view_of(const void* host) {
+        for (const PinnedView* v : {&stage_view, &pinned_view})
+            if (v->dev && (const uint8_t*)host >= v->host && (const uint8_t*)host < v->host + v->bytes) return v->dev + ((const uint8_t*)host - v->host);
+        return device_view(const_cast<void*>(host));
+    }
     void memset(void* p, int v, size_t n) {
+        if (batch_on) { bq.fill(p, n, v); return; }
         if (n >= ((size_t)1 << 20) && ((uintptr_t)p & 15) == 0) {
             const int64_t n16 = (int64_t)(n >> 4);
             const uint32_t w = 0x01010101u * (uint32_t)(uint8_t)v;
@@ -192,6 +225,7 @@
         check(hipMemsetAsync(p, v, n, stream), "hipMemsetAsync");
     }
     void clear_many(const pm::ClearJob* jobs, int n) {
+        if (batch_on) { for (int i = 0; i < n; i++) bq.fill(jobs[i].p, jobs[i].bytes, jobs[i].value); return; }
         FillJobs f; f.n = 0; unsigned int blocks = 0;
         for (int i = 0; i < n; i++) {
             if (!jobs[i].bytes) continue;
@@ -211,6 +245,7 @@
     static bool copy_log() { static const bool on = getenv("PARSNP_COPY_LOG") != nullptr; return on; }
     static double now_us() { return std::chrono::duration<double, std::micro>(std::chrono::steady_clock::now().time_since_epoch()).count(); }
     uint8_t* ring = nullptr; size_t ring_at = 0; static constexpr size_t kRing = (size_t)4 << 20;
+    uint8_t* ring_dev = nullptr; bool ring_dev_asked = false;
     void h2d(void* d, const void* s, size_t n) {
         const double t0 = copy_log() ? now_us() : 0;
         bytes_h2d += n;
@@ -218,14 +253,17 @@
             if (!ring && hipHostMalloc((void**)&ring, kRing, hipHostMallocDefault) != hipSuccess) ring = nullptr;
             if (ring) {
                 const size_t need = (n + 63) & ~(size_t)63;
-                if (ring_at + need > kRing) { check(hipStreamSynchronize(stream), "sync"); ring_at = 0; }
+                if (ring_at + need > kRing) { about_to_enqueue(); check(hipStreamSynchronize(stream), "sync"); ring_at = 0; }
                 memcpy(ring + ring_at, s, n);
-                check(hipMemcpyAsync(d, ring + ring_at, n, hipMemcpyHostToDevice, stream), "hipMemcpy H2D (ring)");
+                if (batch_on && !ring_dev_asked) { ring_dev_asked = true; ring_dev = (uint8_t*)device_view(ring); }
+                if (batch_on && ring_dev) bq.upload(d, ring_dev + ring_at, ring + ring_at, n);
+                else { about_to_enqueue(); check(hipMemcpyAsync(d, ring + ring_at, n, hipMemcpyHostToDevice, stream), "hipMemcpy H2D (ring)"); }
                 ring_at += need;
                 if (copy_log()) fprintf(stderr, "[copy] h2d (ring) %8zu B %8.1f us\n", n, now_us() - t0);
                 return;
             }
         }
+        about_to_enqueue();
         if (n) check(hipMemcpyAsync(d, s, n, hipMemcpyHostToDevice, stream), "hipMemcpy H2D"); check(hipStreamSynchronize(stream), "sync");
         if (copy_log()) fprintf(stderr, "[copy] h2d       %9zu B %8.1f us\n", n, now_us() - t0);
     }
@@ -233,14 +271,15 @@
     struct Landing { void* dst; const uint8_t* at; size_t n; };
     std::vector<Landing> landings;
     void land() { for (const Landing& l : landings) memcpy(l.dst, l.at, l.n); landings.clear(); dring_at = 0; }
-    void drop_landings() { group.n = 0; group_blocks = 0; grouping = false; if (!landings.empty()) { (void)hipStreamSynchronize(stream); landings.clear(); dring_at = 0; } }
+    void drop_landings() { if (!bq.b.empty()) { bind(); about_to_enqueue(); } group.n = 0; group_blocks = 0; grouping = false; if (!landings.empty()) { (void)hipStreamSynchronize(stream); landings.clear(); dring_at = 0; } }
     bool group_copies = true;
     bool grouping = false; CopyJobs group{}; unsigned int group_blocks = 0; uint8_t* dring_dev = nullptr;
     static constexpr size_t kGroupMax = (size_t)4 << 20;
     void d2h_group() { if (group_copies) grouping = true; }
-    void d2h_flush() { flush_group(); }
+    void d2h_flush() { about_to_enqueue(); flush_group(); }
     void flush_group() {
         if (group.n) {
+            about_to_enqueue();
             group.first_block[group.n] = group_blocks;
             hipLaunchKernelGGL(pm_copy_many, dim3(group_blocks), dim3(256), 0, stream, group);
             check(hipGetLastError(), "pm_copy_many");
@@ -253,11 +292,20 @@
         if (!n) return;
         const size_t need = (n + 255) & ~(size_t)255;
         if (!dring && hipHostMalloc((void**)&dring, kDRing, hipHostMallocDefault) != hipSuccess) dring = nullptr;
-        if (grouping && dring && !dring_dev) {
-            void* dp = nullptr;
-            if (hipHostGetDevicePointer(&dp, dring, 0) == hipSuccess && dp) dring_dev = (uint8_t*)dp; else { (void)hipGetLastError(); group_copies = false; grouping = false; }
-        }
-        if (grouping && dring && n <= kGroupMax && dring_at + need <= kDRing) {
+        const bool by_kernel = group_copies && (grouping || batch_on);
+        if (by_kernel && dring && !dring_dev) {
+            dring_dev = (uint8_t*)device_view(dring);
+            if (!dring_dev) { group_copies = false; grouping = false; }
+        }
+        if (batch_on && by_kernel && dring_dev && n <= kGroupMax && dring_at + need <= kDRing) {
+            bq.copy(dring_dev + dring_at, s, n);
+            landings.push_back(Landing{d, dring + dring_at, n});
+            dring_at += need;
+            if (copy_log()) fprintf(stderr, "[copy] d2h_batch %9zu B\n", n);
+            return;
+        }
+        about_to_enqueue();
+        if (grouping && dring && dring_dev && n <= kGroupMax && dring_at + need <= kDRing) {
             if (group.n == CopyJobs::kMax) flush_group();
             group.src[group.n] = s; group.dst[group.n] = dring_dev + dring_at; group.bytes[group.n] = n; group.first_block[group.n] = group_blocks;
             group_blocks += (unsigned int)((n + 65535) >> 16);
@@ -275,18 +323,24 @@
         if (copy_log()) fprintf(stderr, "[copy] d2h_async %9zu B %8.1f us\n", n, now_us() - t0);
     }
     void d2h_async_pinned(void* d, const void* s, size_t n) {
-        bytes_d2h += n; if (n) check(hipMemcpyAsync(d, s, n, hipMemcpyDeviceToHost, stream), "hipMemcpy D2H (pinned)");
+        bytes_d2h += n;
+        if (batch_on && n && n <= kGroupMax) {
+            if (void* dd = view_of(d)) { bq.copy(dd, s, n); return; }
+        }
+        about_to_enqueue();
+        if (n) check(hipMemcpyAsync(d, s, n, hipMemcpyDeviceToHost, stream), "hipMemcpy D2H (pinned)");
     }
     void d2h(void* d, const void* s, size_t n) {
         const double t0 = copy_log() ? now_us() : 0;
         d2h_async(d, s, n); sync();
         if (copy_log()) fprintf(stderr, "[copy] d2h       %9zu B %8.1f us (with the queued work before it)\n", n, now_us() - t0);
     }
-    void sync() { flush_group(); grouping = false; check(hipStreamSynchronize(stream), "hipStreamSynchronize"); land(); }
+    void sync() { about_to_enqueue(); flush_group(); grouping = false; check(hipStreamSynchronize(stream), "hipStreamSynchronize"); land(); }
     void* event_record() {
         hipEvent_t e = nullptr;
         if (!pool.empty()) { e = pool.back(); pool.pop_back(); }
         else if (!check(hipEventCreate(&e), "hipEventCreate")) return nullptr;
+        about_to_enqueue();
         check(hipEventRecord(e, stream), "hipEventRecord");
         return (void*)e;
     }
@@ -295,18 +349,37 @@
     void* stage_p = nullptr; size_t stage_cap = 0;
     void* staging(size_t n) {
         if (n > stage_cap) {
+            if (!bq.b.empty()) { about_to_enqueue(); check(hipStreamSynchronize(stream), "sync"); }
             if (stage_p) (void)hipHostFree(stage_p);
-            stage_p = nullptr; stage_cap = 0;
+            stage_p = nullptr; stage_cap = 0; stage_view = PinnedView{};
             if (!check(hipHostMalloc(&stage_p, n + n / 4 + 4096, hipHostMallocDefault), "hipHostMalloc(staging)")) return nullptr;
             stage_cap = n + n / 4 + 4096;
+            stage_view = PinnedView{(const uint8_t*)stage_p, (uint8_t*)device_view(stage_p), stage_cap};
         }
         return stage_p;
     }
-    void d2d(void* d, const void* s, size_t n) { if (n) check(hipMemcpyAsync(d, s, n, hipMemcpyDeviceToDevice, stream), "hipMemcpy D2D"); }
-    void* pinned_alloc(size_t n) { void* p = nullptr; if (!check(hipHostMalloc(&p, n ? n : 1, hipHostMallocDefault), "hipHostMalloc")) return nullptr; return p; }
-    void pinned_free(void* p) { if (p) (void)hipHostFree(p); }
+    void d2d(void* d, const void* s, size_t n) {
+        if (batch_on) { bq.copy(d, s, n); return; }
+        if (n) check(hipMemcpyAsync(d, s, n, hipMemcpyDeviceToDevice, stream), "hipMemcpy D2D");
+    }
+    void* pinned_alloc(size_t n) {
+        void* p = nullptr;
+        if (!check(hipHostMalloc(&p, n ? n : 1, hipHostMallocDefault), "hipHostMalloc")) return nullptr;
+        pinned_view = PinnedView{(const uint8_t*)p, (uint8_t*)device_view(p), n ? n : 1};
+        return p;
+    }
+    void pinned_free(void* p) {
+        if (p && !bq.b.empty()) { about_to_enqueue(); check(hipStreamSynchronize(stream), "sync"); }
+        if (p && p == (void*)pinned_view.host) pinned_view = PinnedView{};
+        if (p) (void)hipHostFree(p);
+    }
     void h2d_staged(void* d, const void* s, size_t n) {
-        bytes_h2d += n; if (n) check(hipMemcpyAsync(d, s, n, hipMemcpyHostToDevice, stream), "hipMemcpy H2D (staged)");
+        bytes_h2d += n;
+        if (batch_on && n && n <= kUploadKernelMax) {
+            if (void* sd = view_of(s)) { bq.upload(d, sd, s, n); if (getenv("PARSNP_COPY_LOG")) fprintf(stderr, "[copy] h2d_staged %8zu B (table)\n", n); return; }
+        }
+        about_to_enqueue();
+        if (n) check(hipMemcpyAsync(d, s, n, hipMemcpyHostToDevice, stream), "hipMemcpy H2D (staged)");
         if (getenv("PARSNP_COPY_LOG")) fprintf(stderr, "[copy] h2d_staged %8zu B\n", n);
     }
 
@@ -319,6 +392,7 @@
         constexpr int kPer = 2;
         int device = 0;
         if (!check(hipGetDevice(&device), "hipGetDevice")) return false;
+        about_to_enqueue();
         check(hipStreamSynchronize(stream), "sync");
         struct Slot { uint8_t* host = nullptr; uint8_t* dev = nullptr; hipStream_t st = nullptr; hipEvent_t done = nullptr; bool used = false; };
         std::vector<Slot> slots((size_t)kThreads * kPer);
@@ -367,12 +441,14 @@
         if (n <= 0) return;
         int64_t blocks = (n + 255) / 256;
         if (blocks > 0x7fffffffll) { if (err.empty()) err = std::string("grid too large: ") + name; return; }
+        about_to_enqueue();
         hipLaunchKernelGGL(pm_kernel<F>, dim3((unsigned)blocks), dim3(256), 0, stream, f, n);
         check(hipGetLastError(), name);
     }
     template <class F> void launch_wave(const char* name, int64_t n, F f) {
         if (n <= 0) return;
         if (n > 0x7fffffffll) { if (err.empty()) err = std::string("grid too large: ") + name; return; }
+        about_to_enqueue();
         hipLaunchKernelGGL(pm_wave_kernel<F>, dim3((unsigned)n), dim3(64), 0, stream, f, n);
         check(hipGetLastError(), name);
     }
@@ -384,12 +460,14 @@
     }
     void exclusive_scan(const int64_t* in, int64_t* out, size_t n) {
         size_t bytes = 0;
+        about_to_enqueue();
         check(rocprim::exclusive_scan(nullptr, bytes, in, out, (int64_t)0, n, rocprim::plus<int64_t>(), stream), "scan size");
         need_tmp(bytes);
         check(rocprim::exclusive_scan(tmp, bytes, in, out, (int64_t)0, n, rocprim::plus<int64_t>(), stream), "exclusive_scan");
     }
     void sort_pairs(uint64_t* ki, uint64_t* ko, uint64_t* vi, uint64_t* vo, size_t n, int bits) {
         size_t bytes = 0;
+        about_to_enqueue();
         check(rocprim::radix_sort_pairs(nullptr, bytes, ki, ko, vi, vo, n, 0, (unsigned)bits, stream), "sort size");
         need_tmp(bytes);
         check(rocprim::radix_sort_pairs(tmp, bytes, ki, ko, vi, vo, n, 0, (unsigned)bits, stream), "radix_sort_pairs");
@@ -397,6 +475,7 @@
 
     void sort_keys(uint64_t* ki, uint64_t* ko, size_t n, int begin_bit, int end_bit) {
         size_t bytes = 0;
+        about_to_enqueue();
         check(rocprim::radix_sort_keys(nullptr, bytes, ki, ko, n, (unsigned)begin_bit, (unsigned)end_bit, stream), "sort size");
         need_tmp(bytes);
         check(rocprim::radix_sort_keys(tmp, bytes, ki, ko, n, (unsigned)begin_bit, (unsigned)end_bit, stream), "radix_sort_keys");
```

Result: faster. 31740 (median of 6 runs) (+1.8%).
